# in3otd/glfer

Measured on AMD Instinct MI355X. Metric: spectrogram frames/sec + achieved HBM GB/s, N=4096 MTM K=4, higher is better.
Workload: dtype f32

## Files before the change

### glfer_amd/api.py

```python
import ctypes as C
import os

import numpy as np

_HERE = os.path.dirname(os.path.abspath(__file__))
LIB_PATH = os.environ.get("GLFER_LIB_PATH") or os.path.join(_HERE, "lib", "libglfer_hip.so")

MODE_FFT, MODE_MTM, MODE_HPARMA, MODE_LMP = 0, 1, 2, 3
WAV_PARTIAL_TAIL = 1
WINDOWS = {"hanning": 0, "blackman": 1, "gaussian": 2, "welch": 3,
           "bartlett": 4, "rectangular": 5, "hamming": 6, "kaiser": 7}
SAMPLES_F32, SAMPLES_S16, SAMPLES_U8 = 0, 1, 2
HISTORY_ZERO_FIRST, HISTORY_ZERO_ALWAYS = 0, 1
SUBMEAN_OFF, SUBMEAN_EXACT, SUBMEAN_FAST = 0, 1, 2
AVG_SUMAVG, AVG_PLAIN, AVG_SUMEXTREME = 1, 2, 3

EXPORTS = [
    "glfer_hip_plan_create", "glfer_hip_plan_destroy", "glfer_hip_hop", "glfer_hip_bins",
    "glfer_hip_num_tapers", "glfer_hip_num_frames", "glfer_hip_get_window", "glfer_hip_get_tapers",
    "glfer_hip_make_window", "glfer_hip_make_dpss", "glfer_hip_spectrogram_device",
    "glfer_hip_spectrum_device", "glfer_hip_spectrogram_host", "glfer_hip_wav_probe",
    "glfer_hip_spectrogram_wav", "glfer_hip_submean_device",
    "glfer_hip_floor_device",
    "glfer_hip_avg_device", "glfer_hip_palette", "glfer_hip_display_device", "glfer_hip_strerror", "glfer_hip_last_hip_error", "glfer_hip_version",
    "glfer_hip_frame_range", "glfer_hip_prepare_device", "glfer_hip_mtm_ftest_device", "glfer_hip_host_alloc",
    "glfer_hip_host_free", "glfer_hip_spectrogram_host_multi", "glfer_hip_spectrogram_wav_ex",
    "glfer_hip_avg_cum_device", "glfer_hip_waterfall_host", "glfer_hip_waterfall_device",
    "glfer_hip_spectrogram_host_workers",
    "glfer_hip_scratch_trim", "glfer_hip_scratch_held", "glfer_hip_scratch_limit", "glfer_hip_spectrogram_wav_range",
    "glfer_hip_spectrogram_wav_multi", "glfer_hip_spectrogram_wav_workers", "glfer_hip_levels_host",
    "glfer_hip_waterfall_map_device", "glfer_hip_waterfall_host_workers", "glfer_hip_waterfall_wav_workers",
    "glfer_hip_waterfall_wav_multi", "glfer_hip_submean_exact_device",
    "glfer_hip_numa_node_of_bus_id", "glfer_hip_numa_node_cpus", "glfer_hip_floor_device_pitched",
    "glfer_hip_abi_version", "glfer_hip_spectrogram_avg_device", "glfer_hip_workers_create", "glfer_hip_workers_destroy",
    "glfer_hip_workers_spectrogram_wav", "glfer_hip_workers_spectrogram_host",
    "glfer_hip_spectrogram_batch_device", "glfer_hip_avg_batch_device", "glfer_hip_spectrogram_avg_batch_device",
    "glfer_hip_waterfall_batch_device",
]


class GlferHipError(RuntimeError):
    pass


class Config(C.Structure):
    _fields_ = [("mode", C.c_int), ("n", C.c_int), ("overlap", C.c_float),
                ("window_type", C.c_int), ("limiter_a", C.c_float), ("enable_limiter", C.c_int),
                ("sub_mean", C.c_int), ("history_mode", C.c_int), ("mtm_w", C.c_float),
                ("mtm_k", C.c_int), ("sample_format", C.c_int), ("device", C.c_int),
                ("hparma_t", C.c_int), ("hparma_p_e", C.c_int), ("lmp_av", C.c_int), ("psd_pitch", C.c_int)]


class Display(C.Structure):
    _fields_ = [("scale_type", C.c_int), ("autoscale", C.c_int), ("overlap", C.c_float),
                ("max_level_db", C.c_float), ("min_level_db", C.c_float), ("thr_level", C.c_float),
                ("palette", C.c_int), ("first_buffer", C.c_int), ("display_max_lvl", C.c_float),
                ("display_min_lvl", C.c_float), ("psd_pitch", C.c_int)]

    def __init__(self, scale_type=2, autoscale=1, overlap=0.0, max_level_db=-10.0, min_level_db=-60.0,
                 thr_level=0.0, palette=0, first_buffer=1, psd_pitch=0):
        super().__init__(scale_type, autoscale, overlap, max_level_db, min_level_db, thr_level,
                         palette, first_buffer, 0.0, 0.0, psd_pitch)


SCALE_LIN, SCALE_LIN_MAX0, SCALE_LOG, SCALE_LOG_MAX0 = range(4)
PALETTES = {"hsv": 0, "thresh": 1, "cool": 2, "hot": 3, "bw": 4, "bone": 5, "copper": 6, "otd": 7}


class Phases(C.Structure):
    _fields_ = [("setup_s", C.c_double), ("read_s", C.c_double), ("h2d_s", C.c_double), ("kernel_s", C.c_double),
                ("d2h_s", C.c_double), ("wall_s", C.c_double), ("chunks", C.c_uint)]

    def as_dict(self):
        return {k: getattr(self, k) for k, _ in self._fields_}


class WavInfo(C.Structure):
    _fields_ = [("format", C.c_int), ("channels", C.c_int), ("sample_rate", C.c_int),
                ("bits_per_sample", C.c_int), ("data_offset", C.c_size_t), ("nsamples", C.c_size_t),
                ("data_bytes", C.c_size_t)]


_lib = None


def lib():
    global _lib
    if _lib is not None:
        return _lib
    try:
        import torch
    except ImportError:
        pass
    if not os.path.exists(LIB_PATH):
        raise GlferHipError(
            "HIP extension not built: %s is missing (run `python -c 'import __graft_entry__ as g; "
            "g.build()'` or `make -C glfer_amd/csrc`). There is no CPU fallback." % LIB_PATH)
    L = C.CDLL(LIB_PATH)
    vp, sz = C.c_void_p, C.c_size_t
    L.glfer_hip_plan_create.argtypes = [C.POINTER(Config), C.POINTER(vp)]
    L.glfer_hip_plan_destroy.argtypes = [vp]
    L.glfer_hip_plan_destroy.restype = None
    for f in ("glfer_hip_hop", "glfer_hip_bins", "glfer_hip_num_tapers"):
        getattr(L, f).argtypes = [vp]
    L.glfer_hip_num_frames.argtypes = [vp, sz]
    L.glfer_hip_num_frames.restype = sz
    L.glfer_hip_get_window.argtypes = [vp, vp]
    L.glfer_hip_get_tapers.argtypes = [vp, vp, vp]
    L.glfer_hip_make_window.argtypes = [C.c_int, C.c_int, vp]
    L.glfer_hip_make_dpss.argtypes = [C.c_int, C.c_int, C.c_double, vp, vp]
    L.glfer_hip_spectrogram_device.argtypes = [vp, vp, sz, sz, sz, vp, vp]
    L.glfer_hip_spectrogram_batch_device.argtypes = [vp, vp, sz, sz, sz, sz, sz, vp, vp]
    L.glfer_hip_spectrum_device.argtypes = [vp, vp, sz, sz, sz, vp, vp, vp]
    L.glfer_hip_spectrogram_host.argtypes = [vp, vp, sz, vp, C.POINTER(sz)]
    L.glfer_hip_wav_probe.argtypes = [C.c_char_p, C.POINTER(WavInfo)]
    L.glfer_hip_spectrogram_wav.argtypes = [vp, C.c_char_p, vp, sz, C.POINTER(sz), sz]
    L.glfer_hip_submean_device.argtypes = [vp, vp, C.c_int, sz, C.c_int, vp]
    L.glfer_hip_submean_exact_device.argtypes = [vp, vp, C.c_int, sz, C.c_int, vp]
    L.glfer_hip_floor_device.argtypes = [vp, sz, C.c_int, vp, vp]
    L.glfer_hip_floor_device_pitched.argtypes = [vp, sz, C.c_int, C.c_int, vp, vp]
    L.glfer_hip_palette.argtypes = [C.c_int, vp]
    L.glfer_hip_display_device.argtypes = [C.POINTER(Display), vp, vp, vp, sz, C.c_int, vp, vp, vp, vp]
    L.glfer_hip_avg_device.argtypes = [C.c_int, vp, sz, C.c_int, C.c_int, C.c_int, C.c_int, C.c_int,
                                       C.c_int, vp, vp, vp]
    L.glfer_hip_frame_range.argtypes = [sz, C.c_uint, C.c_uint, C.POINTER(sz), C.POINTER(sz)]
    L.glfer_hip_frame_range.restype = None
    L.glfer_hip_prepare_device.argtypes = [vp, vp, sz, sz, sz, vp, vp]
    L.glfer_hip_mtm_ftest_device.argtypes = [vp, vp, sz, sz, sz, vp, C.c_int, vp]
    L.glfer_hip_host_alloc.argtypes = [sz]
    L.glfer_hip_host_alloc.restype = vp
    L.glfer_hip_host_free.argtypes = [vp]
    L.glfer_hip_host_free.restype = None
    L.glfer_hip_spectrogram_host_multi.argtypes = [C.POINTER(Config), C.c_uint, vp, sz, vp, C.POINTER(sz)]
    L.glfer_hip_spectrogram_host_workers.argtypes = [C.POINTER(Config), C.POINTER(C.c_int), C.c_int, vp, sz, vp, C.POINTER(sz)]
    L.glfer_hip_spectrogram_wav_ex.argtypes = [vp, C.c_char_p, vp, sz, C.POINTER(sz), sz, C.c_uint]
    L.glfer_hip_avg_cum_device.argtypes = [vp, sz, C.c_int, C.c_int, C.c_int, C.c_int, C.c_int, vp, vp]
    L.glfer_hip_waterfall_device.argtypes = [C.POINTER(Display), C.c_int, C.c_int, C.c_int, C.c_int, C.c_int, vp, sz, C.c_int,
                                             vp, vp, vp, vp]
    L.glfer_hip_waterfall_host.argtypes = [vp, C.POINTER(Display), vp, sz, vp, vp, C.POINTER(sz)]
    cfgp, ip, dispp, szp = C.POINTER(Config), C.POINTER(C.c_int), C.POINTER(Display), C.POINTER(sz)
    L.glfer_hip_spectrogram_wav_range.argtypes = [vp, C.c_char_p, sz, sz, vp, szp, sz, C.c_uint]
    L.glfer_hip_spectrogram_wav_multi.argtypes = [cfgp, C.c_uint, C.c_char_p, vp, sz, szp, C.c_uint]
    L.glfer_hip_spectrogram_wav_workers.argtypes = [cfgp, ip, C.c_int, C.c_char_p, vp, sz, szp, C.c_uint]
    L.glfer_hip_waterfall_host_workers.argtypes = [cfgp, ip, C.c_int, dispp, C.c_int, C.c_int, C.c_int, C.c_int, C.c_int,
                                                   vp, sz, vp, vp, szp]
    L.glfer_hip_waterfall_wav_workers.argtypes = [cfgp, ip, C.c_int, dispp, C.c_int, C.c_int, C.c_int, C.c_int, C.c_int,
                                                  C.c_char_p, sz, vp, vp, szp, C.c_uint]
    L.glfer_hip_waterfall_wav_multi.argtypes = [cfgp, C.c_uint, dispp, C.c_int, C.c_int, C.c_int, C.c_int, C.c_int,
                                                C.c_char_p, sz, vp, vp, szp, C.c_uint]
    L.glfer_hip_levels_host.argtypes = [dispp, vp, sz, vp, C.c_int]
    L.glfer_hip_waterfall_map_device.argtypes = [dispp, C.c_int, C.c_int, C.c_int, C.c_int, C.c_int, vp, sz, sz, C.c_int,
                                                 vp, vp, vp, vp]
    L.glfer_hip_numa_node_of_bus_id.argtypes = [C.c_char_p, C.c_char_p]
    L.glfer_hip_numa_node_cpus.argtypes = [C.c_int, C.c_char_p, vp, sz]
    L.glfer_hip_scratch_trim.argtypes = [C.c_int, sz]
    L.glfer_hip_scratch_trim.restype = sz
    L.glfer_hip_scratch_held.argtypes = [C.c_int]
    L.glfer_hip_scratch_held.restype = sz
    L.glfer_hip_scratch_limit.argtypes = [sz]
    L.glfer_hip_scratch_limit.restype = None
    for f in ("glfer_hip_strerror", "glfer_hip_last_hip_error", "glfer_hip_version"):
        getattr(L, f).restype = C.c_char_p
    L.glfer_hip_strerror.argtypes = [C.c_int]
    L.glfer_hip_abi_version.argtypes = []
    L.glfer_hip_workers_create.argtypes = [C.POINTER(Config), C.POINTER(C.c_int), C.c_int, sz, C.POINTER(vp)]
    L.glfer_hip_workers_destroy.argtypes = [vp]
    L.glfer_hip_workers_destroy.restype = None
    L.glfer_hip_workers_spectrogram_wav.argtypes = [vp, C.c_char_p, vp, sz, C.POINTER(sz), C.c_uint, C.POINTER(Phases)]
    L.glfer_hip_workers_spectrogram_host.argtypes = [vp, vp, sz, vp, C.POINTER(sz), C.POINTER(Phases)]
    L.glfer_hip_spectrogram_avg_device.argtypes = [vp, vp, sz, sz, sz, C.c_int, C.c_int, C.c_int, C.c_int, C.c_int, C.c_int, vp, vp, vp, vp]
    L.glfer_hip_waterfall_batch_device.argtypes = [dispp, sz, C.c_int, C.c_int, C.c_int, C.c_int, C.c_int, vp, sz, C.c_int, vp, vp,
                                                   vp, vp]
    L.glfer_hip_avg_batch_device.argtypes = [C.c_int, vp, sz, sz, C.c_int, C.c_int, C.c_int, C.c_int, C.c_int, C.c_int, vp, vp, vp]
    L.glfer_hip_spectrogram_avg_batch_device.argtypes = [vp, vp, sz, sz, sz, sz, sz, C.c_int, C.c_int, C.c_int, C.c_int, C.c_int,
                                                         C.c_int, vp, vp, vp, vp]
    _lib = L
    return L


def _check(rc, what):
    if rc != 0:
        L = lib()
        raise GlferHipError("%s failed: %s (%s)" % (
            what, L.glfer_hip_strerror(rc).decode(), L.glfer_hip_last_hip_error().decode()))


def version():
    return lib().glfer_hip_version().decode()


def make_window(window_type, n):
    w = np.empty(n, np.float32)
    _check(lib().glfer_hip_make_window(int(window_type), n, w.ctypes.data), "make_window")
    return w


def make_dpss(n, kmax, nw):
    v = np.empty((kmax + 1, n), np.float64)
    s = np.empty(kmax + 1, np.float64)
    _check(lib().glfer_hip_make_dpss(n, kmax, float(nw), v.ctypes.data, s.ctypes.data), "make_dpss")
    return v, s


class FftParams:

    def __init__(self, n=1024, window_type=7, overlap=0.0, a=0.0, limiter=0, sub_mean=0,
                 history_mode=HISTORY_ZERO_FIRST, sample_format=SAMPLES_F32, psd_pitch=0):
        self.mode = MODE_FFT
        self.psd_pitch = psd_pitch
        self.n, self.window_type, self.overlap = n, window_type, overlap
        self.a, self.limiter, self.sub_mean = a, limiter, sub_mean
        self.history_mode, self.sample_format = history_mode, sample_format
        self.w, self.kmax = 0.0, 0


class MtmParams:

    def __init__(self, n=1024, overlap=0.0, w=4.0, kmax=7, sub_mean=0,
                 history_mode=HISTORY_ZERO_FIRST, sample_format=SAMPLES_F32, psd_pitch=0):
        self.mode = MODE_MTM
        self.psd_pitch = psd_pitch
        self.n, self.overlap, self.w, self.kmax = n, overlap, w, kmax
        self.window_type = WINDOWS["rectangular"]
        self.a, self.limiter, self.sub_mean = 0.0, 0, sub_mean
        self.history_mode, self.sample_format = history_mode, sample_format


class HparmaParams:

    def __init__(self, n=4096, overlap=0.0, t=96, p_e=16, sub_mean=0, history_mode=HISTORY_ZERO_FIRST,
                 sample_format=SAMPLES_F32):
        self.mode = MODE_HPARMA
        self.n, self.overlap, self.t, self.p_e = n, overlap, t, p_e
        self.window_type = WINDOWS["rectangular"]
        self.a, self.limiter, self.sub_mean = 0.0, 0, sub_mean
        self.history_mode, self.sample_format = history_mode, sample_format
        self.w, self.kmax = 0.0, 0


class LmpParams:

    def __init__(self, n=1024, overlap=0.0, avg=4, sub_mean=0, history_mode=HISTORY_ZERO_FIRST,
                 sample_format=SAMPLES_F32):
        self.mode = MODE_LMP
        self.n, self.overlap, self.avg = n, overlap, avg
        self.window_type = WINDOWS["rectangular"]
        self.a, self.limiter, self.sub_mean = 0.0, 0, sub_mean
        self.history_mode, self.sample_format = history_mode, sample_format
        self.w, self.kmax = 0.0, 0


_TORCH_DTYPES = None


def _torch():
    import torch
    return torch


def make_config(params, device=0):
    return Config(params.mode, params.n, params.overlap, params.window_type, params.a,
                  params.limiter, params.sub_mean, params.history_mode, params.w, params.kmax,
                  params.sample_format, device, getattr(params, "t", 0), getattr(params, "p_e", 0),
# ... 438 lines not shown
```

### glfer_amd/csrc/glfer_hip.cpp

```cpp
#include "plan.h"

#include <algorithm>
#include <cmath>
#include <cstdlib>
#include <cstdio>
#include <cstring>
#include <map>
#include <mutex>
#include <new>

#include "host_tables.h"
#include "spectro_params.h"

extern "C" hipError_t glfer_launch_hparma(const SpectroParams *sp, int n, int t, int ncol, const int *rot_sched, int rot_steps, int rot_width, const uint16_t *lagmap,
                                          const float2 *unit, hipStream_t st);
extern "C" hipError_t glfer_launch_floor(const float *psd, size_t nframes, int bins, int pitch, int m, float *stats,
                                         hipStream_t st);
extern "C" hipError_t glfer_launch_avg(int mode, const float *psd, size_t nframes, int bins, int n_out,
                                       int depth, int minbin, int maxbin, int max0, double *avg,
                                       double *ret, hipStream_t st);
extern "C" hipError_t glfer_launch_avg_batch(int mode, const float *psd, size_t nframes, int bins, int n_out, int depth, int minbin,
                                             int maxbin, int max0, double *avg, double *ret, unsigned nb, long long psd_bs,
                                             long long avg_bs, long long ret_bs, hipStream_t st);
extern "C" int glfer_avgmap_applies(size_t walk, int bins, int depth, int minbin, int maxbin);
// ... 149 lines not shown
      } else if (!b.out && b.cap >= want && (!best || b.cap < best->cap)) {
        best = &b;
      }
    }
    if (!best && !empty) {
      BigBlock *victim = nullptr;
      for (BigBlock &b : ds.big)
        if (!b.out && b.cap < want && (!victim || b.cap < victim->cap)) victim = &b;
      if (victim) {
        drop_block(*victim);
        empty = victim;
      }
    }
    if (!best && empty) {
      size_t held = 0;
      for (BigBlock &b : ds.big)
        if (b.p) held += b.cap;
      if (held + want > g_scratch_cap) trim_locked(ds, g_scratch_cap > want ? g_scratch_cap - want : 0);
      void *q = nullptr;
      hipEvent_t ev = nullptr;
      hipError_t me = hipMalloc(&q, want);
      if (me != hipSuccess) {
        (void)hipGetLastError();
        q = nullptr;
        if (trim_locked(ds, 0) > 0) me = hipMalloc(&q, want);
        for (BigBlock &b : ds.big)
          if (!b.p) { empty = &b; break; }
      }
      if (me == hipSuccess && hipEventCreateWithFlags(&ev, hipEventDisableTiming) == hipSuccess) {
        empty->p = q;
        empty->cap = want;
        empty->freed = ev;
        empty->used = false;
        empty->dev = dev;
        best = empty;
      } else {
        (void)hipGetLastError();
        if (q) (void)hipFree(q);
      }
    }
    if (best) {
      best->out = true;
      hipError_t e = hipSuccess;
      if (best->used && best->last != st) e = hipStreamWaitEvent(st, best->freed, 0);
      if (e != hipSuccess) {
        best->out = false;
        return e;
      }
      *p = best->p;
      return hipSuccess;
    }
  }
  lock.unlock();
  return hipMallocAsync(p, bytes, st);
}

void scratch_free(void *q, hipStream_t st) {
  if (!q) return;
  {
    std::lock_guard<std::mutex> lock(g_scratch_mu);
    for (DeviceScratch &ds : g_scratch)
      for (BigBlock &b : ds.big)
        if (b.p == q) {
          int cur = -1;
          const bool moved = hipGetDevice(&cur) == hipSuccess && cur != b.dev && b.dev >= 0 && hipSetDevice(b.dev) == hipSuccess;
          if (hipEventRecord(b.freed, st) == hipSuccess) {
            b.used = true;
            b.last = st;
          } else {
            (void)hipGetLastError();
            if (hipStreamSynchronize(st) != hipSuccess) {
              (void)hipGetLastError();
              (void)hipDeviceSynchronize();
              (void)hipFree(b.p);
              (void)hipEventDestroy(b.freed);
              b = BigBlock();
              if (moved) (void)hipSetDevice(cur);
              return;
            }
            b.used = false;
            b.last = nullptr;
          }
          b.out = false;
          if (b.dev >= 0 && b.dev < 64) trim_locked(g_scratch[b.dev], g_scratch_cap);
          if (moved) (void)hipSetDevice(cur);
          return;
        }
  }
  (void)hipFreeAsync(q, st);
}

size_t scratch_trim(int dev, size_t keep_bytes) {
  if (dev < 0 || dev >= 64) return 0;
  DeviceGuard guard(dev);
  std::lock_guard<std::mutex> lock(g_scratch_mu);
  return trim_locked(g_scratch[dev], keep_bytes);
}
size_t scratch_held(int dev) {
  if (dev < 0 || dev >= 64) return 0;
  std::lock_guard<std::mutex> lock(g_scratch_mu);
  size_t held = 0;
  for (BigBlock &b : g_scratch[dev].big)
    if (b.p) held += b.cap;
  return held;
}
void scratch_set_cap(size_t bytes) {
  std::lock_guard<std::mutex> lock(g_scratch_mu);
  g_scratch_cap = bytes;
  int cur = -1;
  if (hipGetDevice(&cur) != hipSuccess) cur = -1;
  for (int dev = 0; dev < 64; dev++) {
    size_t held = 0;
    for (BigBlock &b : g_scratch[dev].big)
      if (b.p) held += b.cap;
    if (held <= bytes) continue;
    if (dev != cur && hipSetDevice(dev) != hipSuccess) { (void)hipGetLastError(); continue; }
    trim_locked(g_scratch[dev], bytes);
    if (dev != cur && cur >= 0) (void)hipSetDevice(cur);
  }
}

hipError_t allow_dynamic_lds(const void *kernel, size_t bytes) {
  static std::mutex mu;
  static std::map<std::pair<int, const void *>, size_t> allowed;
  int dev = 0;
  hipError_t e = hipGetDevice(&dev);
  if (e != hipSuccess) return e;
  std::lock_guard<std::mutex> lock(mu);
  size_t &have = allowed[{dev, kernel}];
  if (bytes <= have) return hipSuccess;
  e = hipFuncSetAttribute(kernel, hipFuncAttributeMaxDynamicSharedMemorySize, (int)bytes);
  if (e == hipSuccess) have = bytes;
  return e;
}

}
using glfer::DeviceGuard;
using glfer::hip_fail;

static int data_device(const void *d_ptr) {
  int dev = glfer::device_of(d_ptr);
  if (dev < 0 && hipGetDevice(&dev) != hipSuccess) dev = 0;
  return dev;
}

static bool is_pow2(int n) { return n > 0 && (n & (n - 1)) == 0; }

static size_t tap_slot(int n, int pair, int i, int which) {
  if (n < 256) return ((size_t)pair * n + i) * 2 + which;
  const int T = n / 16, t = i % T, m = i / T;
  return (size_t)pair * n * 2 + ((size_t)(m / 2) * T + t) * 4 + (size_t)(m & 1) * 2 + which;
}

extern "C" {

const char *glfer_hip_version(void) { return "glfer_hip 0.9 (gfx950; 16 points/lane Stockham radix-16 with LDS exchange, inter-pass twiddles folded into the butterflies: packed pairs, real-input and wavefront-private forms, shared odd taper, register reuse across overlapped frames, mean removal in the reference's summation order (cfg.sub_mean = 1) or inside the kernels; N = 8..1048576; periodogram, multitaper + F-test, HP-ARMA with column-disjoint Jacobi rotations side by side and frames from a queue, LMP; rows at a caller's pitch; wavefront floor, fused average, display map with the average taken inside it; chunk ring for ingest with uploads and downloads at once, WAV files and waterfalls over several GPUs, read-ahead behind the per-hop shim, kept scratch blocks with a cap, workers bound to their GPU's NUMA node)"; }

int glfer_hip_abi_version(void) { return GLFER_HIP_ABI; }

int glfer_hip_palette(int palette, unsigned char colortab[768]) {
  if (!colortab) return GLFER_E_ARG;
  glfer::make_palette(palette, colortab);
  return GLFER_OK;
}

}

struct MapAverages {
  int mode, depth, minbin, maxbin, max0;
  const float *d_batch;
  size_t first;
};

static int display_columns(glfer_hip_display *d, const float *d_psd, const double *d_avg, const MapAverages *fused,
                           const float *d_stats, size_t nframes, int bins, unsigned char *d_rgb, short *d_lev,
                           float *d_levels, void *hip_stream, const float *d_levels_in = nullptr, int psd_pitch = 0) {
  if (!d || (!d_stats && !d_levels_in) || !d_rgb || bins < 1) return GLFER_E_ARG;
  if (psd_pitch == 0) psd_pitch = bins;
  if (psd_pitch < bins || (fused && psd_pitch != bins)) return GLFER_E_ARG;
  if ((d_psd != nullptr) + (d_avg != nullptr) + (fused != nullptr) != 1) return GLFER_E_ARG;
  if (d->scale_type < GLFER_SCALE_LIN || d->scale_type > GLFER_SCALE_LOG_MAX0) return GLFER_E_ARG;
  if (nframes == 0) return GLFER_OK;
  hipStream_t st = (hipStream_t)hip_stream;
  DeviceGuard guard(data_device(d_rgb));
  HIP_TRY(guard.error());
  const int scale_log = d->scale_type == GLFER_SCALE_LOG || d->scale_type == GLFER_SCALE_LOG_MAX0;

  const size_t lev_floats = (d_levels || d_levels_in) ? 0 : nframes * 4;
  const size_t st_floats = (d->autoscale && !d_levels_in) ? glfer_levels_scratch_floats(nframes) : 0;
  const size_t thr_bytes = (2 * glfer::kLogThrK + 1) * sizeof(double);
  unsigned char *scratch = nullptr;
  HIP_TRY(glfer::scratch_malloc((void **)&scratch, 768 + thr_bytes + (lev_floats + st_floats) * sizeof(float), st));
  unsigned char *d_tab = scratch;
  double *d_thr = reinterpret_cast<double *>(scratch + 768);
  float *fs = reinterpret_cast<float *>(scratch + 768 + thr_bytes);
  float *levels = d_levels_in ? const_cast<float *>(d_levels_in) : (d_levels ? d_levels : fs);
  float *chunk_state = st_floats ? fs + lev_floats : nullptr;
  int rc = GLFER_OK;
  auto fail = [&](hipError_t err) { rc = hip_fail(err, "glfer_hip_display_device"); };
  unsigned char tab[768];
  glfer::make_palette(d->palette, tab);
  hipError_t e = hipMemcpyAsync(d_tab, tab, 768, hipMemcpyHostToDevice, st);
  if (e == hipSuccess) e = hipMemcpyAsync(d_thr, glfer::log_thresholds(), thr_bytes, hipMemcpyHostToDevice, st);
  if (e != hipSuccess) fail(e);

  if (rc == GLFER_OK && !d_levels_in) {
    if (d->autoscale) {
      e = glfer_launch_levels(d_stats, nframes, scale_log, 1, d->first_buffer, d->overlap, d->display_max_lvl,
                              d->display_min_lvl, levels, chunk_state, st);
    } else {
      float mx = pow(10.0, d->max_level_db / 10.0);
      float mn = pow(10.0, d->min_level_db / 10.0);
      mn = (mx > mn ? mn : mx / 10.0);
      const float dmax = scale_log ? (float)(10.0 * log10(mx)) : mx;
      const float dmin = scale_log ? (float)(10.0 * log10(mn)) : mn;
      e = glfer_launch_levels_fixed(nframes, dmax, dmin, mx, mn, levels, st);
    }
    if (e != hipSuccess) fail(e);
  }
  if (rc == GLFER_OK) {
    const float thr_level = d->thr_level / 100.0;
    if (fused)
      e = glfer_launch_avgmap(fused->mode, fused->d_batch, fused->first, fused->first + nframes, bins, fused->depth,
                              fused->minbin, fused->maxbin, fused->max0, scale_log, 255.0 * thr_level,
                              1.0 - thr_level, levels, d_tab, d_thr, d_rgb, d_lev, st);
    else
      e = glfer_launch_map(d_psd, d_avg, nframes, bins, psd_pitch, scale_log, 255.0 * thr_level, 1.0 - thr_level, levels,
                           d_tab, d_thr, d_rgb, d_lev, st);
    if (e != hipSuccess) fail(e);
  }
  float last[4] = {0, 0, 0, 0};
  if (rc == GLFER_OK && !d_levels_in) {
    e = hipMemcpyAsync(last, levels + (nframes - 1) * 4, sizeof last, hipMemcpyDeviceToHost, st);
    if (e != hipSuccess) fail(e);
  }
  glfer::scratch_free(scratch, st);
  e = hipStreamSynchronize(st);
  if (e != hipSuccess && rc == GLFER_OK) fail(e);
  if (rc == GLFER_OK && !d_levels_in) {
    d->display_max_lvl = last[2];
    d->display_min_lvl = last[3];
    if (d->autoscale) d->first_buffer = 0;
  }
  return rc;
}

extern "C" {

int glfer_hip_display_device(glfer_hip_display *d, const float *d_psd, const double *d_avg, const float *d_stats,
                             size_t nframes, int bins, unsigned char *d_rgb, short *d_lev, float *d_levels,
                             void *hip_stream) {
  if (!d || (d_psd == nullptr) == (d_avg == nullptr)) return GLFER_E_ARG;
  return display_columns(d, d_psd, d_avg, nullptr, d_stats, nframes, bins, d_rgb, d_lev, d_levels, hip_stream, nullptr, d->psd_pitch);
}

}

static void waterfall_route(int avg_mode, int depth, int minbin, int maxbin, int bins, int pitch, size_t nframes, bool *fused_out,
                            size_t *tile_out) {
  const bool averaging = avg_mode != 0;
  bool fused = averaging && pitch == bins;
  if (const char *e = getenv("GLFER_WATERFALL_FUSED")) fused = fused && atoi(e) != 0;
  size_t tile = (averaging && !fused) ? std::max<size_t>(16384, ((size_t)4 << 30) / ((size_t)bins * sizeof(double))) : (size_t)1 << 22;
  if (const char *e = getenv("GLFER_WATERFALL_TILE")) {
    const long v = atol(e);
    if (v >= 64) tile = (size_t)v;
  }
  tile = std::min(tile, nframes);
  tile = (nframes + (nframes + tile - 1) / tile - 1) / ((nframes + tile - 1) / tile);
  const size_t last_tile = nframes - (nframes - 1) / tile * tile;
  if (fused) fused = glfer_avgmap_applies(tile, bins, depth, minbin, maxbin) != 0 &&
                     glfer_avgmap_applies(last_tile, bins, depth, minbin, maxbin) != 0;
  *fused_out = fused;
  *tile_out = tile;
}

static int waterfall_columns(glfer_hip_display *d, int avg_mode, int depth, int minbin, int maxbin, int max0,
                             const float *d_batch, size_t row0, size_t nframes, int bins, unsigned char *d_rgb, short *d_lev,
                             float *d_stats, void *hip_stream, const float *d_levels_in, int pitch = 0) {
  if (pitch == 0) pitch = bins;
  const float *d_psd = d_batch ? d_batch + row0 * (size_t)pitch : nullptr;
  if (!d || !d_psd || !d_rgb || bins < 1 || bins > 32769 || pitch < bins) return GLFER_E_ARG;
  const bool averaging = avg_mode != 0;
  if (averaging && (avg_mode < GLFER_AVG_SUMAVG || avg_mode > GLFER_AVG_SUMEXTREME || depth < 1 || minbin < 0 ||
                    maxbin <= minbin || maxbin > bins))
    return GLFER_E_ARG;
  if (nframes == 0) return GLFER_OK;
  hipStream_t st = (hipStream_t)hip_stream;
  DeviceGuard guard(data_device(d_psd));
  HIP_TRY(guard.error());
  bool fused = false;
  size_t tile = 0;
  waterfall_route(avg_mode, depth, minbin, maxbin, bins, pitch, nframes, &fused, &tile);
  const size_t back = averaging ? (size_t)depth : 0;
  float *stats = d_stats;
  double *avg = nullptr, *ret = nullptr;
  if (!stats && !d_levels_in) HIP_TRY(glfer::scratch_malloc((void **)&stats, tile * 4 * sizeof(float), st));
  int rc = GLFER_OK;
  if (averaging && !fused) {
    hipError_t e = glfer::scratch_malloc((void **)&avg, (tile + back) * (size_t)bins * sizeof(double), st);
    if (e == hipSuccess) e = glfer::scratch_malloc((void **)&ret, (tile + back) * 4 * sizeof(double), st);
    if (e != hipSuccess) rc = hip_fail(e, "hipMallocAsync(waterfall tile)");
  }
  for (size_t f0 = 0; rc == GLFER_OK && f0 < nframes; f0 += tile) {
    const size_t nf = std::min(tile, nframes - f0);
    float *tstats = d_stats ? d_stats + f0 * 4 : stats;
// ... 237 lines not shown
  if (ret) glfer::scratch_free(ret, st);
  if (levels) glfer::scratch_free(levels, st);
  if (!d_stats && stats) glfer::scratch_free(stats, st);
  glfer::scratch_free(small, st);
  e = hipStreamSynchronize(st);
  if (e != hipSuccess) fail(e, "glfer_hip_waterfall_batch_device");
  if (rc == GLFER_OK) {
    for (size_t b = 0; b < nstreams; b++) {
      if (autoscale) {
        disps[b].display_max_lvl = back_state[b * 3 + 1];
        disps[b].display_min_lvl = back_state[b * 3 + 2];
        disps[b].first_buffer = 0;
      } else {
        disps[b].display_max_lvl = mx;
        disps[b].display_min_lvl = mn;
      }
    }
  }
  return rc;
}

size_t glfer_hip_scratch_trim(int device, size_t keep_bytes) {
  size_t ring = 0;
  if (keep_bytes == 0 && device >= 0 && device < 64) {
    DeviceGuard guard(device);
    if (guard.error() == hipSuccess) {
      ring = glfer::workers_kept_bytes(device);
      glfer::workers_drop_kept();
      ring += glfer::ingest_ring_spare_bytes(device);
      glfer::ingest_ring_drop_spare(device);
    }
  }
  return ring + glfer::scratch_trim(device, keep_bytes);
}
size_t glfer_hip_scratch_held(int device) { return glfer::scratch_held(device) + glfer::ingest_ring_spare_bytes(device) + glfer::workers_kept_bytes(device); }
void glfer_hip_scratch_limit(size_t bytes) {
  glfer::scratch_set_cap(bytes);
  if (bytes == 0) glfer::workers_drop_kept();
  int cur = -1;
  if (hipGetDevice(&cur) != hipSuccess) cur = -1;
  for (int dev = 0; dev < 64; dev++)
    if (glfer::ingest_ring_spare_bytes(dev) > bytes) {
      DeviceGuard guard(dev);
      if (guard.error() == hipSuccess) glfer::ingest_ring_drop_spare(dev);
    }
}

const char *glfer_hip_strerror(int code) {
  switch (code) {
    case GLFER_OK: return "ok";
    case GLFER_E_ARG: return "bad argument or unsupported configuration";
    case GLFER_E_HIP: return "HIP runtime error";
    case GLFER_E_NOMEM: return "out of memory";
    case GLFER_E_NUMERIC: return "DPSS eigen-solve did not converge";
  }
  return "unknown error";
}

const char *glfer_hip_last_hip_error(void) { return g_hip_err.c_str(); }

int glfer_hip_plan_create(const glfer_hip_config *cfg, glfer_hip_plan **out) {
  if (!cfg || !out) return GLFER_E_ARG;
  *out = nullptr;
  const int n = cfg->n;
  if (!is_pow2(n) || n < 8 || n > (1 << 20)) return GLFER_E_ARG;
  if (cfg->mode == GLFER_MODE_HPARMA && (n < 32 || n > 32768)) return GLFER_E_ARG;
  const bool small = n < 256, huge = n > 16384;
  if (!(cfg->overlap >= 0.0f) || !(cfg->overlap < 1.0f)) return GLFER_E_ARG;
  if (cfg->mode != GLFER_MODE_FFT && cfg->mode != GLFER_MODE_MTM && cfg->mode != GLFER_MODE_HPARMA &&
      cfg->mode != GLFER_MODE_LMP)
    return GLFER_E_ARG;
  if (cfg->mode == GLFER_MODE_LMP && (cfg->lmp_av < 1 || cfg->lmp_av > 4096)) return GLFER_E_ARG;
  if (cfg->mode == GLFER_MODE_HPARMA) {
    const int t = cfg->hparma_t, ncol = cfg->hparma_p_e + 1;
    if (t < 2 || ncol < 2 || ncol > t || t > n || ncol > 256 || t > 65535) return GLFER_E_ARG;
    const size_t xlen = (size_t)n + (t <= 128 ? 128 : 0);
    const size_t big = xlen > (size_t)t * ncol ? xlen : (size_t)t * ncol;
    if ((big + (size_t)ncol * ncol + t + 2 * ncol) * sizeof(float) > 160 * 1024) return GLFER_E_ARG;
  }
  if (cfg->sample_format < 0 || cfg->sample_format > 2) return GLFER_E_ARG;
  if (cfg->mode == GLFER_MODE_MTM && (cfg->mtm_k < 0 || cfg->mtm_k > 31 || !(cfg->mtm_w > 0.0f)))
    return GLFER_E_ARG;
  if (cfg->mode == GLFER_MODE_FFT && (cfg->window_type < 0 || cfg->window_type > 7)) return GLFER_E_ARG;

  glfer_hip_plan *p = new (std::nothrow) glfer_hip_plan();
  if (!p) return GLFER_E_NOMEM;
  p->cfg = *cfg;
  p->n = n;
  p->hop = (int)(n * (1.0 - cfg->overlap));
  p->keep = n - p->hop;
  p->bins = n / 2 + 1;
  p->lanes = n / 64;
  if (p->hop <= 0) { delete p; return GLFER_E_ARG; }
  p->pitch = cfg->psd_pitch ? cfg->psd_pitch : p->bins;
  if (cfg->psd_pitch < 0 || p->pitch < p->bins || (cfg->psd_pitch && cfg->mode == GLFER_MODE_LMP)) { delete p; return GLFER_E_ARG; }

  p->window.assign(n, 1.0f);
  std::vector<float> taps;
  const bool lmp = cfg->mode == GLFER_MODE_LMP;
  if (lmp) {
    p->cfg.window_type = GLFER_WIN_RECTANGULAR;
    p->cfg.limiter_a = 0.0f;
    p->cfg.enable_limiter = 0;
    p->lmp_av = cfg->lmp_av;
  }
  if (cfg->mode == GLFER_MODE_FFT || lmp) {
    p->ntapers = 1;
    p->npairs = 1;
    glfer::make_window(p->cfg.window_type, n, p->window.data());
    p->nonlin = (p->cfg.limiter_a > 0.0f) || (p->cfg.enable_limiter == 1);
    const double scale = std::sqrt(1.0 / ((huge ? 4.0 : 2.0) * n));
    p->spec_unscale = (float)scale;
    taps.assign((size_t)2 * n, 0.0f);
    const bool rect = (p->cfg.window_type == GLFER_WIN_RECTANGULAR);
    for (int i = 0; i < n; i++) {
      const double w = rect ? 1.0 : (double)p->window[i];
      taps[tap_slot(n, 0, i, 0)] = p->nonlin ? (float)w : (float)(w * scale);
    }
  } else if (cfg->mode == GLFER_MODE_HPARMA) {
    p->ntapers = 0;
    p->npairs = 0;
    taps.assign(4, 0.0f);
  } else {
    p->ntapers = cfg->mtm_k + 1;
    p->npairs = (p->ntapers + 1) / 2;
    p->tapers.resize((size_t)p->ntapers * n);
    p->sig.resize(p->ntapers);
    {
      struct Kept { int n, kmax; float w; std::vector<double> tapers, sig; };
      static std::mutex mu;
      static std::vector<Kept> kept;
      bool hit = false;
      {
        std::lock_guard<std::mutex> lock(mu);
        for (const Kept &k : kept)
          if (k.n == n && k.kmax == cfg->mtm_k && k.w == cfg->mtm_w) {
            p->tapers = k.tapers;
            p->sig = k.sig;
            hit = true;
            break;
          }
      }
      if (!hit) {
        if (!glfer::make_dpss(n, cfg->mtm_k, (double)cfg->mtm_w, p->tapers.data(), p->sig.data())) {
          delete p;
          return GLFER_E_NUMERIC;
        }
        std::lock_guard<std::mutex> lock(mu);
        if (kept.size() >= 4) kept.erase(kept.begin());
        kept.push_back(Kept{n, cfg->mtm_k, cfg->mtm_w, p->tapers, p->sig});
      }
    }
    taps.assign((size_t)2 * p->npairs * n, 0.0f);
    for (int j = 0; j < p->ntapers && !huge; j++) {
      const double scale = std::sqrt(1.0 / (2.0 * n * (1.0 + p->sig[j])));
      for (int i = 0; i < n; i++)
        taps[tap_slot(n, j / 2, i, j & 1)] = (float)(p->tapers[(size_t)j * n + i] * scale);
    }
    p->spec_unscale = 1.0f;
  }
  int logn = 0;
  while ((1 << logn) < n) logn++;
  p->lanes = n / 16;
  std::vector<float> tw(2, 0.0f);
  if (!small && !huge) {
    tw.assign((size_t)2 * glfer::make_twiddles16(logn, nullptr) * p->lanes, 0.0f);
    glfer::make_twiddles16(logn, tw.data());
  }
  if (huge) taps.assign(4, 0.0f);

  std::vector<float> htaps, htw, hrot;
  const bool h_periodogram = (cfg->mode == GLFER_MODE_FFT || lmp) && !p->nonlin && n >= 512 && !huge;
  const bool h_multitaper = cfg->mode == GLFER_MODE_MTM && n >= 8192 && !huge;
  if (h_periodogram || h_multitaper) {
    const int th = n / 32;
    const int nwin = h_multitaper ? p->ntapers : 1;
    const bool rect = h_periodogram && (p->cfg.window_type == GLFER_WIN_RECTANGULAR);
    htaps.resize((size_t)nwin * n);
    for (int j = 0; j < nwin; j++) {
      const double scale = std::sqrt(1.0 / (4.0 * n * (h_multitaper ? 1.0 + p->sig[j] : 1.0)));
      for (int m = 0; m < 16; m++)
        for (int t = 0; t < th; t++)
          for (int e = 0; e < 2; e++) {
            const int i = 2 * (t + th * m) + e;
            const double w = h_multitaper ? p->tapers[(size_t)j * n + i] : (rect ? 1.0 : (double)p->window[i]);
            htaps[(size_t)j * n + ((size_t)(m / 2) * th + t) * 4 + (size_t)(m & 1) * 2 + e] = (float)(w * scale);
          }
    }
    p->htapers = nwin;
    htw.resize((size_t)2 * glfer::make_twiddles16(logn - 1, nullptr) * th);
    glfer::make_twiddles16(logn - 1, htw.data());
    hrot.resize((size_t)2 * th);
    for (int t = 0; t < th; t++) {
      const double ang = 2.0 * 3.14159265358979323846 * t / n;
      hrot[2 * t] = (float)std::cos(ang);
      hrot[2 * t + 1] = (float)std::sin(ang);
    }
  }

  std::vector<float> wtaps, wtw, wcomb;
  const bool w_form = (((cfg->mode == GLFER_MODE_FFT || lmp) && (!p->nonlin || huge)) || cfg->mode == GLFER_MODE_MTM) && n >= 2048;
  if (w_form) {
    const int M = n / 2, W = M / 1024, LF = 64 * W, IPL = LF <= 512 ? 512 / LF : 1;
    const bool mt = cfg->mode == GLFER_MODE_MTM;
    const int nwin = mt ? p->ntapers : 1;
    const bool rect = !mt && (p->cfg.window_type == GLFER_WIN_RECTANGULAR);
    wtaps.resize((size_t)nwin * n);
    for (int j = 0; j < nwin; j++) {
      const double scale = std::sqrt(1.0 / (4.0 * n * (mt ? 1.0 + p->sig[j] : 1.0)));
      for (int w = 0; w < W; w++)
        for (int m = 0; m < 16; m++)
          for (int t = 0; t < 64; t++)
            for (int e = 0; e < 2; e++) {
              const int i = 2 * (W * (t + 64 * m) + w) + e;
              const double v = mt ? p->tapers[(size_t)j * n + i] : (rect ? 1.0 : (double)p->window[i]);
              wtaps[((((size_t)j * W + w) * 8 + m / 2) * 64 + t) * 4 + (size_t)(m & 1) * 2 + e] = (float)(p->nonlin ? v : v * scale);
            }
    }
    p->wtapers = nwin;
    wtw.resize((size_t)2 * glfer::make_twiddles16(10, nullptr) * 64);
    glfer::make_twiddles16(10, wtw.data());
    wcomb.resize(n <= 32768 ? (size_t)2 * IPL * W * LF : 2);
    const double two_pi = 2.0 * 3.14159265358979323846;
    for (int i = 0; i < IPL && n <= 32768; i++)
      for (int ww = 0; ww < W; ww++)
        for (int u = 0; u < LF; u++) {
          const long long k1 = u + (long long)LF * i;
          const double ang = ww == 0 ? two_pi * (double)k1 / n : two_pi * (double)((ww * k1) % M) / M;
          wcomb[2 * ((size_t)(i * W + ww) * LF + u)] = (float)std::cos(ang);
          wcomb[2 * ((size_t)(i * W + ww) * LF + u) + 1] = (float)std::sin(ang);
        }
  }

  std::vector<float> xtaps;
  if (cfg->mode == GLFER_MODE_MTM && (p->ntapers & 1) && p->ntapers >= 3 && !small && !huge) {
    const int T = n / 16, j = p->ntapers - 1;
    const double scale = std::sqrt(1.0 / (4.0 * n * (1.0 + p->sig[j])));
    xtaps.resize((size_t)n);
    for (int i = 0; i < n; i++) {
      const int t = i % T, m = i / T;
      xtaps[((size_t)(m / 4) * T + t) * 4 + (size_t)(m & 3)] = (float)(p->tapers[(size_t)j * n + i] * scale);
    }
  }

  std::vector<float> ltaps;
  if (!xtaps.empty() && n <= 4096) {
    const int T = n / 16, nfull = p->npairs - 1;
    bool sym = true;
    for (int j = 0; j < p->ntapers && sym; j++) {
      const double *v = &p->tapers[(size_t)j * n];
      double peak = 0.0, dev = 0.0;
      for (int i = 0; i < n / 2; i++) {
        peak = std::max(peak, std::fabs(v[i]));
        dev = std::max(dev, std::fabs(v[n - 1 - i] - ((j & 1) ? -v[i] : v[i])));
      }
      sym = dev <= 1e-7 * peak;
    }
    const size_t lds = ((size_t)(n + n / 16) * (T >= 256 ? 1 : 256 / T) + 16 * 17 + 8 + (size_t)nfull * 8 * T + 4 * T) * 8;
    if (sym && lds <= 80 * 1024) {
      ltaps.resize((size_t)nfull * 8 * T * 2 + (size_t)8 * T);
      for (int j = 0; j < p->ntapers; j++) {
        const bool last = j == p->ntapers - 1;
        const double scale = std::sqrt(1.0 / ((last ? 4.0 : 2.0) * n * (1.0 + p->sig[j])));
        for (int m = 0; m < 8; m++)
          for (int t = 0; t < T; t++) {
            const float val = (float)(p->tapers[(size_t)j * n + t + T * m] * scale);
            if (last) ltaps[(size_t)nfull * 8 * T * 2 + (size_t)m * T + t] = val;
            else ltaps[(((size_t)(j / 2) * 8 + m) * T + t) * 2 + (j & 1)] = val;
          }
      }
    }
  }

  std::vector<uint16_t> lagmap;
  std::vector<float> unit;
  std::vector<int> rot_sched;
  if (cfg->mode == GLFER_MODE_HPARMA) {
    const int t = cfg->hparma_t, ncol = cfg->hparma_p_e + 1;
    const int width = [] { const char *e = getenv("GLFER_HPARMA_WIDTH"); return e && atoi(e) == 16 ? 16 : 8; }();
    p->rot_width = width;
    if (ncol >= 2 && ncol <= 64) {
      std::vector<std::pair<int, int>> rots;
      for (int j = 0; j < ncol - 1; j++)
        for (int k = j + 1; k < ncol; k++) rots.push_back({j, k});
      const int R = (int)rots.size();
      std::vector<std::vector<int>> succ(R);
      std::vector<int> indeg(R, 0), lastc(ncol, -1), lp(R, 1);
      for (int i = 0; i < R; i++) {
        const int cs[2] = {rots[i].first, rots[i].second};
        int seen = -1;
        for (int c : cs) {
          if (lastc[c] >= 0 && lastc[c] != seen) {
            succ[lastc[c]].push_back(i);
            indeg[i]++;
            seen = lastc[c];
          }
          lastc[c] = i;
        }
      }
      for (int i = R - 1; i >= 0; i--)
        for (int s : succ[i]) lp[i] = std::max(lp[i], 1 + lp[s]);
      std::vector<int> ready;
      for (int i = 0; i < R; i++)
        if (!indeg[i]) ready.push_back(i);
      int done = 0;
      while (done < R) {
        std::sort(ready.begin(), ready.end(), [&](int a, int b) { return lp[a] != lp[b] ? lp[a] > lp[b] : a < b; });
        const int take = std::min<int>(width, (int)ready.size());
        std::vector<int> cur(ready.begin(), ready.begin() + take);
        ready.erase(ready.begin(), ready.begin() + take);
        for (int g = 0; g < width; g++) rot_sched.push_back(g < take ? (rots[cur[g]].first | rots[cur[g]].second << 8) : -1);
        for (int i : cur) {
          done++;
          for (int s : succ[i])
            if (--indeg[s] == 0) ready.push_back(s);
        }
      }
    }
    std::vector<int> flat((size_t)(t + 1) * ncol, -1);
    for (int i = 0; i < t; i++) flat[i] = i;
    for (int i = 1; i < t; i++)
      for (int j = 0; j < ncol; j++) flat[(size_t)i * ncol + j] = flat[std::abs(j - i)];
    lagmap.resize((size_t)t * ncol);
    for (size_t i = 0; i < lagmap.size(); i++) lagmap[i] = (uint16_t)(flat[i] < 0 ? 0 : flat[i]);
    unit.resize((size_t)2 * (n / 2 + 1));
    for (int k = 0; k <= n / 2; k++) {
      const double ang = -2.0 * 3.14159265358979323846 * k / n;
      unit[2 * k] = (float)std::cos(ang);
      unit[2 * k + 1] = (float)std::sin(ang);
    }
  }

  DeviceGuard guard(cfg->device);
  hipError_t e = guard.error();
  if (e == hipSuccess) e = hipMalloc((void **)&p->d_taps, taps.size() * sizeof(float));
  if (e == hipSuccess && cfg->mode == GLFER_MODE_FFT && cfg->window_type != GLFER_WIN_RECTANGULAR) {
    e = hipMalloc((void **)&p->d_window, (size_t)n * sizeof(float));
    if (e == hipSuccess) e = hipMemcpy(p->d_window, p->window.data(), (size_t)n * sizeof(float), hipMemcpyHostToDevice);
  }
  if (e == hipSuccess) e = hipMalloc((void **)&p->d_tw, tw.size() * sizeof(float));
  if (e == hipSuccess) e = hipMemcpy(p->d_taps, taps.data(), taps.size() * sizeof(float), hipMemcpyHostToDevice);
  if (e == hipSuccess) e = hipMemcpy(p->d_tw, tw.data(), tw.size() * sizeof(float), hipMemcpyHostToDevice);
  if (e == hipSuccess && !htaps.empty()) {
    e = hipMalloc((void **)&p->d_htaps, htaps.size() * sizeof(float));
    if (e == hipSuccess) e = hipMalloc((void **)&p->d_htw, htw.size() * sizeof(float));
    if (e == hipSuccess) e = hipMalloc((void **)&p->d_hrot, hrot.size() * sizeof(float));
    if (e == hipSuccess) e = hipMemcpy(p->d_htaps, htaps.data(), htaps.size() * sizeof(float), hipMemcpyHostToDevice);
    if (e == hipSuccess) e = hipMemcpy(p->d_htw, htw.data(), htw.size() * sizeof(float), hipMemcpyHostToDevice);
    if (e == hipSuccess) e = hipMemcpy(p->d_hrot, hrot.data(), hrot.size() * sizeof(float), hipMemcpyHostToDevice);
  }
  if (e == hipSuccess && !wtaps.empty()) {
    e = hipMalloc((void **)&p->d_wtaps, wtaps.size() * sizeof(float));
    if (e == hipSuccess) e = hipMalloc((void **)&p->d_wtw, wtw.size() * sizeof(float));
    if (e == hipSuccess) e = hipMalloc((void **)&p->d_wcomb, wcomb.size() * sizeof(float));
    if (e == hipSuccess) e = hipMemcpy(p->d_wtaps, wtaps.data(), wtaps.size() * sizeof(float), hipMemcpyHostToDevice);
    if (e == hipSuccess) e = hipMemcpy(p->d_wtw, wtw.data(), wtw.size() * sizeof(float), hipMemcpyHostToDevice);
    if (e == hipSuccess) e = hipMemcpy(p->d_wcomb, wcomb.data(), wcomb.size() * sizeof(float), hipMemcpyHostToDevice);
    if (e == hipSuccess && huge) {
      const int M = n / 2, W = M / 1024;
      std::vector<float> bt((size_t)W * 16 * 2);
      for (int w = 0; w < W; w++)
        for (int m = 0; m < 16; m++) {
          const double ang = -2.0 * 3.14159265358979323846 * (double)(((long long)64 * w * m) % M) / M;
          bt[2 * ((size_t)w * 16 + m)] = (float)std::cos(ang);
          bt[2 * ((size_t)w * 16 + m) + 1] = (float)std::sin(ang);
        }
      e = hipMalloc((void **)&p->d_bigtw, bt.size() * sizeof(float));
      if (e == hipSuccess) e = hipMemcpy(p->d_bigtw, bt.data(), bt.size() * sizeof(float), hipMemcpyHostToDevice);
    }
  }
  if (e == hipSuccess && !xtaps.empty()) {
    e = hipMalloc((void **)&p->d_xtaps, xtaps.size() * sizeof(float));
    if (e == hipSuccess) e = hipMemcpy(p->d_xtaps, xtaps.data(), xtaps.size() * sizeof(float), hipMemcpyHostToDevice);
  }
  if (e == hipSuccess && !ltaps.empty()) {
    e = hipMalloc((void **)&p->d_ltaps, ltaps.size() * sizeof(float));
    if (e == hipSuccess) e = hipMemcpy(p->d_ltaps, ltaps.data(), ltaps.size() * sizeof(float), hipMemcpyHostToDevice);
  }
  if (e == hipSuccess && !lagmap.empty()) {
    e = hipMalloc((void **)&p->d_lagmap, lagmap.size() * sizeof(uint16_t));
    if (e == hipSuccess) e = hipMalloc((void **)&p->d_unit, unit.size() * sizeof(float));
    if (e == hipSuccess) e = hipMemcpy(p->d_lagmap, lagmap.data(), lagmap.size() * sizeof(uint16_t), hipMemcpyHostToDevice);
    if (e == hipSuccess && !rot_sched.empty()) {
      e = hipMalloc((void **)&p->d_rot_sched, rot_sched.size() * sizeof(int));
      if (e == hipSuccess) e = hipMemcpy(p->d_rot_sched, rot_sched.data(), rot_sched.size() * sizeof(int), hipMemcpyHostToDevice);
      p->rot_steps = (int)(rot_sched.size() / p->rot_width);
    }
    if (e == hipSuccess) e = hipMemcpy(p->d_unit, unit.data(), unit.size() * sizeof(float), hipMemcpyHostToDevice);
  }
  if (e != hipSuccess) {
    int rc = hip_fail(e, "plan_create");
    glfer_hip_plan_destroy(p);
    return rc;
  }
  *out = p;
  return GLFER_OK;
}

void glfer_hip_plan_destroy(glfer_hip_plan *p) {
  if (!p) return;
  DeviceGuard guard(p->cfg.device);
  if (p->d_taps) (void)hipFree(p->d_taps);
  if (p->d_window) (void)hipFree(p->d_window);
  if (p->d_ftaps_mu_first) (void)hipFree(p->d_ftaps_mu_first);
  if (p->d_ftaps2) (void)hipFree(p->d_ftaps2);
  if (p->d_U0) (void)hipFree(p->d_U0);
  if (p->d_tw) (void)hipFree(p->d_tw);
  if (p->d_htaps) (void)hipFree(p->d_htaps);
  if (p->d_htw) (void)hipFree(p->d_htw);
  if (p->d_hrot) (void)hipFree(p->d_hrot);
  if (p->d_xtaps) (void)hipFree(p->d_xtaps);
  if (p->d_wtaps) (void)hipFree(p->d_wtaps);
  if (p->d_wtw) (void)hipFree(p->d_wtw);
  if (p->d_wcomb) (void)hipFree(p->d_wcomb);
  if (p->d_bigtw) (void)hipFree(p->d_bigtw);
  if (p->d_ltaps) (void)hipFree(p->d_ltaps);
  if (p->d_lagmap) (void)hipFree(p->d_lagmap);
  if (p->d_rot_sched) (void)hipFree(p->d_rot_sched);
  if (p->d_unit) (void)hipFree(p->d_unit);
  glfer::ingest_ring_free(p->ring);
  for (hipStream_t a : p->aux)
    if (a) (void)hipStreamDestroy(a);
  for (hipEvent_t ev : p->aux_events) (void)hipEventDestroy(ev);
  delete p;
}

int glfer_hip_hop(const glfer_hip_plan *p) { return p ? p->hop : GLFER_E_ARG; }
int glfer_hip_bins(const glfer_hip_plan *p) { return p ? p->bins : GLFER_E_ARG; }
int glfer_hip_num_tapers(const glfer_hip_plan *p) { return p ? p->ntapers : GLFER_E_ARG; }
size_t glfer_hip_num_frames(const glfer_hip_plan *p, size_t nsamples) {
  return p ? nsamples / (size_t)p->hop : 0;
}

int glfer_hip_get_window(const glfer_hip_plan *p, float *w) {
  if (!p || !w) return GLFER_E_ARG;
  memcpy(w, p->window.data(), (size_t)p->n * sizeof(float));
  return GLFER_OK;
}

int glfer_hip_get_tapers(const glfer_hip_plan *p, double *tapers, double *sig) {
  if (!p || p->cfg.mode != GLFER_MODE_MTM) return GLFER_E_ARG;
  if (tapers) memcpy(tapers, p->tapers.data(), p->tapers.size() * sizeof(double));
  if (sig) memcpy(sig, p->sig.data(), p->sig.size() * sizeof(double));
  return GLFER_OK;
}

int glfer_hip_make_window(int window_type, int n, float *window) {
  if (!window || n < 2 || window_type < 0 || window_type > 7) return GLFER_E_ARG;
  glfer::make_window(window_type, n, window);
  return GLFER_OK;
}

int glfer_hip_make_dpss(int n, int kmax, double nw, double *tapers, double *sig) {
  if (!tapers || !sig || n < 2 || kmax < 0 || kmax > 31 || !(nw > 0.0)) return GLFER_E_ARG;
  return glfer::make_dpss(n, kmax, nw, tapers, sig) ? GLFER_OK : GLFER_E_NUMERIC;
}

extern "C" hipError_t glfer_launch_spectro_small(const SpectroParams *p, int n, const float *staps, hipStream_t st);
extern "C" hipError_t glfer_launch_spectro16w_n15(const SpectroParams *p, hipStream_t st);
extern "C" hipError_t glfer_launch_spectro_big(const SpectroParams *p, int n, hipStream_t st);

static hipError_t launch_packed(const SpectroParams &sp, int n, hipStream_t st) {
  if (n < 256) return glfer_launch_spectro_small(&sp, n, sp.taps, st);
  switch (n) {
    case 256: return glfer_launch_spectro16_n8(&sp, st);
    case 512: return glfer_launch_spectro16_n9(&sp, st);
    case 1024: return glfer_launch_spectro16_n10(&sp, st);
    case 2048: return glfer_launch_spectro16_n11(&sp, st);
    case 4096: return glfer_launch_spectro16_n12(&sp, st);
    case 8192: return glfer_launch_spectro16_n13(&sp, st);
    case 16384: return glfer_launch_spectro16_n14(&sp, st);
  }
  return hipErrorInvalidValue;
}

static hipError_t launch_real_input(const SpectroParams &sp, int n, hipStream_t st) {
  switch (n) {
    case 512: return glfer_launch_spectro16h_n9(&sp, st);
    case 1024: return glfer_launch_spectro16h_n10(&sp, st);
    case 2048: return glfer_launch_spectro16h_n11(&sp, st);
    case 4096: return glfer_launch_spectro16h_n12(&sp, st);
    case 8192: return glfer_launch_spectro16h_n13(&sp, st);
    case 16384: return glfer_launch_spectro16h_n14(&sp, st);
  }
  return hipErrorInvalidValue;
}

#define GLFER_W_PERIODOGRAM(n) (false)
#define GLFER_W_MULTITAPER(n, tapers) ((n) >= 16384)

static int form_override();

static hipError_t launch_wave_private(const SpectroParams &sp, int n, hipStream_t st) {
  switch (n) {
    case 2048: return glfer_launch_spectro16w_n11(&sp, st);
    case 4096: return glfer_launch_spectro16w_n12(&sp, st);
    case 8192: return glfer_launch_spectro16w_n13(&sp, st);
    case 16384: return glfer_launch_spectro16w_n14(&sp, st);
    case 32768: return (sp.spec || form_override() == 'w') ? glfer_launch_spectro16w_n15(&sp, st) : glfer_launch_spectro_big(&sp, n, st);
    case 65536: return glfer_launch_spectro_big(&sp, n, st);
  }
  if (n >= 131072 && n <= (1 << 20)) return glfer_launch_spectro_big(&sp, n, st);
  return hipErrorInvalidValue;
}

static int form_override() {
  const char *e = getenv("GLFER_FORM");
  return e && *e ? (int)*e : 0;
}

static hipError_t launch_shared_odd(const SpectroParams &sp, int n, hipStream_t st) {
  if (n == 4096) return glfer_launch_spectro16y_n12(&sp, st);
  if (sp.ltaps) {
    switch (n) {
      case 256: return glfer_launch_spectro16xl_n8(&sp, st);
      case 512: return glfer_launch_spectro16xl_n9(&sp, st);
      case 1024: return glfer_launch_spectro16xl_n10(&sp, st);
      case 2048: return glfer_launch_spectro16xl_n11(&sp, st);
    }
  }
  switch (n) {
    case 256: return glfer_launch_spectro16x_n8(&sp, st);
    case 512: return glfer_launch_spectro16x_n9(&sp, st);
    case 1024: return glfer_launch_spectro16x_n10(&sp, st);
  }
  return hipErrorInvalidValue;
}

enum BodyRoute { ROUTE_PACKED, ROUTE_REAL_INPUT, ROUTE_SHARED_ODD, ROUTE_WAVE_PRIVATE };
static BodyRoute body_route(const SpectroParams &sp, int n) {
  const unsigned esz = sp.fmt == GLFER_FMT_F32 ? 4u : (sp.fmt == GLFER_FMT_S16 ? 2u : 1u);
  const bool pairs_aligned = sp.fmt == GLFER_FMT_F32 ||
                             ((sp.H & 1) == 0 && (reinterpret_cast<uintptr_t>(sp.stream) & (2u * esz - 1u)) == 0);
  const int force = form_override();
  bool real_input = sp.htaps && (sp.npairs == 1 || sp.htapers > 1) && n >= 512 && pairs_aligned;
  bool shared_odd = sp.xtaps && sp.npairs >= 2 && (sp.ltaps || n <= 1024 || n == 4096);
  bool wave_private = sp.wtaps && n >= 2048 && pairs_aligned &&
                      (force == 'w' || (force == 0 && (sp.npairs == 1 ? GLFER_W_PERIODOGRAM(n) : GLFER_W_MULTITAPER(n, sp.wtapers))));
  if (force == 'h') wave_private = false;
  if (force == 'x') wave_private = real_input = false;
  if (wave_private) real_input = true, shared_odd = false;
  if (sp.spec || sp.nonlin || !(real_input || shared_odd)) return ROUTE_PACKED;
  if (wave_private) return ROUTE_WAVE_PRIVATE;
  return real_input ? ROUTE_REAL_INPUT : ROUTE_SHARED_ODD;
}
static bool route_takes_mean(BodyRoute r, const SpectroParams &sp, int n) {
  if (n < 256 || n > 16384 || sp.spec || sp.nonlin || sp.history_mode) return false;
  if ((16 * sp.H) % n) return false;
  const int k16 = 16 * sp.H / n;
  switch (r) {
    case ROUTE_PACKED: return k16 == 4 || k16 == 8 || k16 == 16;
    case ROUTE_REAL_INPUT: return (sp.npairs == 1 && sp.htapers <= 1 && (k16 == 2 || k16 == 4 || k16 == 8 || k16 == 16)) ||
                                  (sp.htapers > 1 && n >= 8192 && k16 == 16);
    case ROUTE_SHARED_ODD: return (n == 4096 || n <= 1024) && (k16 == 4 || k16 == 8 || k16 == 16);
    case ROUTE_WAVE_PRIVATE: return sp.wtapers > 1 && (k16 == 8 || k16 == 16);
    default: return false;
  }
}

static bool route_takes_table(BodyRoute r, const SpectroParams &sp, int n) {
  switch (r) {
    case ROUTE_PACKED: return true;
    case ROUTE_REAL_INPUT: return true;
    case ROUTE_SHARED_ODD: return true;
    case ROUTE_WAVE_PRIVATE: return true;
    default: return false;
  }
}

static hipError_t launch_by_n(const SpectroParams &sp, int n, hipStream_t st) {
  if (n > 16384) return launch_wave_private(sp, n, st);
  const BodyRoute route = body_route(sp, n);
  const bool real_input = route == ROUTE_REAL_INPUT || route == ROUTE_WAVE_PRIVATE, wave_private = route == ROUTE_WAVE_PRIVATE;
  if (sp.mean_inkernel && !route_takes_mean(route, sp, n)) return hipErrorInvalidValue;
  if (route == ROUTE_PACKED) return launch_packed(sp, n, st);
  const long long first_inside = ((long long)sp.R + sp.H - 1) / sp.H;
  if (sp.mean_inkernel && sp.frame0 < first_inside) return hipErrorInvalidValue;
  const int lanes = n / 16;
  const long long G = real_input ? 1 : 2 * (lanes >= 256 ? 1 : 256 / lanes);
  const long long lo = sp.frame0, hi = sp.frame0 + sp.nframes;
  long long b0 = lo > first_inside ? lo : first_inside;
  b0 = (b0 + G - 1) / G * G;
  long long b1 = hi / G * G;
  if (sp.mean_inkernel && (b0 != lo || b1 != hi)) return hipErrorInvalidValue;
  if (b0 >= b1) return launch_packed(sp, n, st);
  auto sub = [&](long long from, long long to) {
    SpectroParams q = sp;
    q.frame0 = from;
    q.nframes = (int)(to - from);
    q.psd = sp.psd + (size_t)(from - lo) * (size_t)sp.pitch;
    q.mean_inkernel = 0;
    q.means = nullptr;
    return q;
  };
  if (b0 > lo) {
    const SpectroParams head = sub(lo, b0);
    hipError_t e = launch_packed(head, n, st);
    if (e != hipSuccess) return e;
  }
  if (hi > b1) {
    const SpectroParams tail = sub(b1, hi);
    hipError_t e = launch_packed(tail, n, st);
    if (e != hipSuccess) return e;
  }
  SpectroParams body = sub(b0, b1);
  body.mean_inkernel = sp.mean_inkernel;
  body.means = sp.means;
  if (wave_private) return launch_wave_private(body, n, st);
  return real_input ? launch_real_input(body, n, st) : launch_shared_odd(body, n, st);
}

}

static void fill_params(const glfer_hip_plan *p, SpectroParams &sp) {
  memset(&sp, 0, sizeof sp);
  sp.H = p->hop;
  sp.R = p->keep;
  sp.npairs = p->npairs;
  sp.history_mode = p->cfg.history_mode ? 1 : 0;
  sp.pitch = p->pitch;
  sp.fmt = p->cfg.sample_format;
  sp.nonlin = p->nonlin ? 1 : 0;
  sp.limiter = (p->cfg.enable_limiter == 1);
  sp.a = p->cfg.limiter_a;
  sp.post_scale = p->spec_unscale;
  sp.spec_unscale = p->spec_unscale;
  sp.taps = p->d_taps;
  sp.tw = p->d_tw;
  sp.htaps = p->d_htaps;
  sp.htapers = p->htapers;
  sp.htw = p->d_htw;
  sp.hrot = p->d_hrot;
  sp.xtaps = p->d_xtaps;
  sp.ltaps = p->d_ltaps;
  sp.wtaps = p->d_wtaps;
  sp.wtapers = p->wtapers;
  sp.wtw = p->d_wtw;
  sp.wcomb = p->d_wcomb;
  sp.bigtw = p->d_bigtw;
}

static bool reference_means(const glfer_hip_plan *p) { return p->cfg.sub_mean != 0 && p->cfg.sub_mean != GLFER_SUBMEAN_FAST; }

static int submean_scratch(const glfer_hip_plan *p, SpectroParams &sp, size_t first, size_t nframes, hipStream_t st,
                           float **scratch_out, long tail_fresh = -1) {
  const size_t hops_back = sp.history_mode ? 0 : (size_t)((p->keep + p->hop - 1) / p->hop);
  size_t hop_lo = (first > hops_back) ? first - hops_back : 0;
  const size_t last = first + nframes - 1;
  if (tail_fresh >= 0 && last > 0 && hop_lo > last - 1) hop_lo = last - 1;
  const size_t nhops = first + nframes - hop_lo;
  float *scratch = nullptr;
  HIP_TRY(glfer::scratch_malloc((void **)&scratch, nhops * (size_t)p->hop * sizeof(float), st));
  const size_t esz = sp.fmt == GLFER_FMT_F32 ? 4 : (sp.fmt == GLFER_FMT_S16 ? 2 : 1);
  const char *src = (const char *)sp.stream + hop_lo * (size_t)p->hop * esz;
  const bool exact = reference_means(p);
  float *means = nullptr;
  hipError_t e = hipSuccess;
  if (exact) {
    e = glfer::scratch_malloc((void **)&means, nhops * sizeof(float), st);
    if (e == hipSuccess) e = glfer_launch_hop_means_seq(src, means, p->hop, (long long)nhops, sp.fmt, st);
  }
  if (e == hipSuccess) e = glfer_launch_submean(src, scratch, p->hop, (long long)nhops, sp.fmt, st, means);
  if (e == hipSuccess && tail_fresh >= 0)
    e = glfer_launch_submean_tail_ex(src + (nhops - 1) * (size_t)p->hop * esz, nhops > 1 ? scratch + (nhops - 2) * (size_t)p->hop : nullptr,
                                     scratch + (nhops - 1) * (size_t)p->hop, p->hop, (int)tail_fresh, exact ? 1 : 0, sp.fmt, st);
  if (means) glfer::scratch_free(means, st);
  if (e != hipSuccess) {
    glfer::scratch_free(scratch, st);
    return hip_fail(e, "glfer_launch_submean");
  }
  sp.stream = reinterpret_cast<const char *>(scratch) - hop_lo * (size_t)p->hop * sizeof(float);
  sp.fmt = GLFER_FMT_F32;
  *scratch_out = scratch;
  return GLFER_OK;
}

static bool mean_inkernel_ok(const glfer_hip_plan *p, const SpectroParams &sp, const float *d_spec, long tail_fresh) {
  if (p->nonlin || d_spec || tail_fresh >= 0 || sp.history_mode) return false;
  if (p->cfg.mode != GLFER_MODE_FFT && p->cfg.mode != GLFER_MODE_LMP && p->cfg.mode != GLFER_MODE_MTM) return false;
  const char *e = getenv("GLFER_MEAN_PREPASS");
  if (e && *e == '1') return false;
  const BodyRoute r = body_route(sp, p->n);
  if (!route_takes_mean(r, sp, p->n)) return false;
  if (reference_means(p) && !route_takes_table(r, sp, p->n)) return false;
  return true;
}

static hipError_t launch_reference_means(const glfer_hip_plan *p, const SpectroParams &sp, size_t hop_lo, size_t nhops, float *means,
                                         unsigned blocks, hipStream_t st) {
  const size_t esz = sp.fmt == GLFER_FMT_F32 ? 4 : (sp.fmt == GLFER_FMT_S16 ? 2 : 1);
  const char *src = (const char *)sp.stream + hop_lo * (size_t)p->hop * esz;
  const int forced = [] { const char *e = getenv("GLFER_MEANS_HPW"); return e && *e ? atoi(e) : 0; }();
  int hpw = forced;
  if (!hpw) hpw = nhops >= 262144 ? (p->hop <= 2048 ? 16 : 64) : (nhops >= 32768 || p->hop % 1024 != 0 ? 16 : 4);
  if (hpw == 4 && p->hop % 1024 != 0) hpw = 16;
  if (hpw == 16 && p->hop % 256 != 0) hpw = 64;
  if ((hpw == 16 || hpw == 4) && (reinterpret_cast<uintptr_t>(src) & (4 * esz - 1)) == 0)
    return glfer_launch_hop_means_tiled(src, means, p->hop, (long long)nhops, sp.fmt, hpw, blocks, st);
  return glfer_launch_hop_means_seq(src, means, p->hop, (long long)nhops, sp.fmt, st);
}

static int launch_body_with_reference_means(glfer_hip_plan *p, const SpectroParams &bs, size_t b0, size_t b1, hipStream_t st) {
  const long piece_mb = [] { const char *e = getenv("GLFER_EXACT_PIECE_MB"); return e && *e ? atol(e) : 0L; }();
  const int nstreams_env = [] {
    const char *e = getenv("GLFER_EXACT_STREAMS");
    const int v = e && *e ? atoi(e) : 2;
    return v < 1 ? 1 : (v > 3 ? 3 : v);
  }();
  const unsigned means_blocks = [] { const char *e = getenv("GLFER_MEANS_BLOCKS"); return e && *e ? (unsigned)atol(e) : 0u; }();
  const size_t hops_back = (size_t)((p->keep + p->hop - 1) / p->hop);
  const size_t hop_lo = b0 - hops_back, nhops = b1 - hop_lo;
  const size_t esz = bs.fmt == GLFER_FMT_F32 ? 4 : (bs.fmt == GLFER_FMT_S16 ? 2 : 1);
  size_t piece = b1 - b0;
  if (piece_mb > 0) {
    piece = ((size_t)piece_mb << 20) / ((size_t)p->hop * esz);
    piece = std::max<size_t>(piece / 64 * 64, 64);
  }
  const size_t npieces = (b1 - b0 + piece - 1) / piece;
  int nstreams = npieces > 1 ? nstreams_env : 1;
  float *means = nullptr;
  hipError_t e = glfer::scratch_malloc((void **)&means, nhops * sizeof(float), st);
  if (e != hipSuccess) return hip_fail(e, "scratch (hop means)");
  SpectroParams q = bs;
  q.means = means - hop_lo;
  {
    const long producers = [] { const char *e = getenv("GLFER_MEANS_PRODUCERS"); return e && *e ? atol(e) : 0L; }();
    const bool periodogram_table = body_route(bs, p->n) == ROUTE_REAL_INPUT && bs.npairs == 1 && bs.htapers <= 1 && p->n <= 8192;
    const long min_frames = [] { const char *e = getenv("GLFER_FUSED_MIN_FRAMES"); return e && *e ? atol(e) : 65536L; }();
    if (producers > 0 && periodogram_table && npieces == 1 && (long)(b1 - b0) >= min_frames) {
      const long block_frames = [] { const char *e = getenv("GLFER_FUSED_BLOCK_FRAMES"); return e && *e ? atol(e) : 0L; }();
      const long look = [] { const char *e = getenv("GLFER_FUSED_LOOK"); return e && *e ? atol(e) : 1024L; }();
      const bool lockstep = block_frames > 0;
      const int chunk = lockstep ? 64 : 4096;
      const size_t nchunks = (nhops + chunk - 1) / chunk;
      unsigned *ready = nullptr;
      e = glfer::scratch_malloc((void **)&ready, (nchunks + 8) * sizeof(unsigned), st);
      if (e == hipSuccess) e = hipMemsetAsync(ready, 0, (nchunks + 8) * sizeof(unsigned), st);
      if (e == hipSuccess) {
        q.nprod = (int)(producers / 8 * 8);
        q.prod_chunk = chunk;
        q.means_out = means - hop_lo;
        q.means_ready = ready;
        q.prod_hop0 = (long long)hop_lo;
        q.prod_nhops = (long long)nhops;
        if (lockstep) {
          q.prod_front_frames = -1;
          q.prod_block_frames = (int)block_frames;
          q.prod_look = (int)look;
          q.front_done = ready + nchunks;
        }
        e = launch_by_n(q, p->n, st);
      }
      if (ready) glfer::scratch_free(ready, st);
      glfer::scratch_free(means, st);
      return e == hipSuccess ? GLFER_OK : hip_fail(e, "estimator launch (hop means produced in the launch)");
    }
  }
  static std::mutex aux_mu;
  bool own_aux = false;
  if (nstreams > 1) {
    std::lock_guard<std::mutex> lock(aux_mu);
    if (p->aux_busy) {
      nstreams = 1;
    } else {
      for (int i = 0; i < nstreams - 1 && e == hipSuccess; i++)
        if (!p->aux[i]) e = hipStreamCreateWithFlags(&p->aux[i], hipStreamNonBlocking);
      while (e == hipSuccess && p->aux_events.size() < 2 * npieces + 1) {
        hipEvent_t ev = nullptr;
        e = hipEventCreateWithFlags(&ev, hipEventDisableTiming);
        if (e == hipSuccess) p->aux_events.push_back(ev);
      }
      if (e != hipSuccess) {
        (void)hipGetLastError();
        nstreams = 1;
        e = hipSuccess;
      } else {
        p->aux_busy = own_aux = true;
      }
    }
  }
  if (nstreams <= 1) {
    for (size_t c = 0; c < npieces && e == hipSuccess; c++) {
      const size_t f0 = b0 + c * piece, f1 = std::min(b1, f0 + piece);
      const size_t h0 = c == 0 ? hop_lo : f0;
      e = launch_reference_means(p, bs, h0, f1 - h0, means + (h0 - hop_lo), 0, st);
      q.frame0 = (long long)f0;
      q.nframes = (int)(f1 - f0);
// ... 255 lines not shown
  const size_t esz = fmt == GLFER_FMT_F32 ? 4 : (fmt == GLFER_FMT_S16 ? 2 : 1);
  if (fmt != GLFER_FMT_F32 && (stream_pitch & 1)) return GLFER_E_ARG;
  const size_t rows = (size_t)p->pitch;
  if (stream_pitch > (SIZE_MAX / esz) / nstreams || nframes > (SIZE_MAX / sizeof(float) / rows) / nstreams) return GLFER_E_ARG;
  return batch_rows(p, d_streams, nstreams, stream_pitch, nsamples, first, nframes, d_psd, nframes * rows, (hipStream_t)hip_stream);
}

static int batch_rows(glfer_hip_plan *p, const void *d_streams, size_t nstreams, size_t stream_pitch, size_t nsamples, size_t first,
                      size_t nframes, float *d_psd, size_t psd_bs, hipStream_t st) {
  const int fmt = p->cfg.sample_format;
  const size_t esz = fmt == GLFER_FMT_F32 ? 4 : (fmt == GLFER_FMT_S16 ? 2 : 1);
  const char *base = static_cast<const char *>(d_streams);
  if (!batch_one_launch(p) || nstreams == 1) {
    for (size_t b = 0; b < nstreams; b++) {
      const int rc = glfer_run_device(p, base + b * stream_pitch * esz, nsamples, first, nframes, d_psd + b * psd_bs, nullptr, st);
      if (rc != GLFER_OK) return rc;
    }
    return GLFER_OK;
  }
  DeviceGuard guard(p->cfg.device);
  HIP_TRY(guard.error());
  int dev = 0, ymax = 0;
  HIP_TRY(hipGetDevice(&dev));
  HIP_TRY(hipDeviceGetAttribute(&ymax, hipDeviceAttributeMaxGridDimY, dev));
  ymax = std::max(1, std::min(ymax, 65535));
  for (size_t c0 = 0; c0 < nstreams; c0 += (size_t)ymax) {
    const unsigned nb = (unsigned)std::min(nstreams - c0, (size_t)ymax);
    SpectroParams sp;
    fill_params(p, sp);
    sp.stream = base + c0 * stream_pitch * esz;
    sp.frame0 = (long long)first;
    sp.nframes = (int)nframes;
    sp.psd = d_psd + c0 * psd_bs;
    sp.nbatch = (int)nb;
    sp.batch_stride = (long long)(stream_pitch * esz);
    sp.psd_batch_stride = (long long)psd_bs;
    int rc = GLFER_OK;
    if (p->cfg.sub_mean && mean_inkernel_ok(p, sp, nullptr, -1)) {
      rc = batch_mean_inkernel(p, sp, first, nframes, nb, st);
    } else {
      float *scratch = nullptr;
      if (p->cfg.sub_mean) rc = batch_submean_scratch(p, sp, first, nframes, nb, st, &scratch);
      if (rc == GLFER_OK) {
        const hipError_t e = launch_by_n(sp, p->n, st);
        if (e != hipSuccess) rc = hip_fail(e, "estimator launch (batch)");
      }
      if (scratch) glfer::scratch_free(scratch, st);
    }
    if (rc != GLFER_OK) return rc;
  }
  return GLFER_OK;
}

int glfer_hip_spectrum_device(glfer_hip_plan *p, const void *d_stream, size_t nsamples, size_t first,
                              size_t nframes, float *d_psd, float *d_spec, void *hip_stream) {
  if (!d_spec) return GLFER_E_ARG;
  return glfer_run_device(p, d_stream, nsamples, first, nframes, d_psd, d_spec, (hipStream_t)hip_stream);
}

int glfer_hip_prepare_device(glfer_hip_plan *p, const void *d_stream, size_t nsamples, size_t first,
                             size_t nframes, float *d_frames, void *hip_stream) {
  if (!p || !d_stream || (!d_frames && nframes)) return GLFER_E_ARG;
  if (nframes == 0) return GLFER_OK;
  if ((first + nframes) > nsamples / (size_t)p->hop || nframes > 0x7fffffffu) return GLFER_E_ARG;
  hipStream_t st = (hipStream_t)hip_stream;
  DeviceGuard guard(p->cfg.device);
  HIP_TRY(guard.error());
  SpectroParams sp;
  fill_params(p, sp);
  sp.stream = d_stream;
  sp.frame0 = (long long)first;
  sp.nframes = (int)nframes;
  float *scratch = nullptr;
  int rc = GLFER_OK;
  if (p->cfg.sub_mean) rc = submean_scratch(p, sp, first, nframes, st, &scratch);
  if (rc == GLFER_OK) {
    hipError_t e = glfer_launch_prepare(&sp, p->n, p->d_window, d_frames, st);
    if (e != hipSuccess) rc = hip_fail(e, "glfer_launch_prepare");
  }
  if (scratch) glfer::scratch_free(scratch, st);
  return rc;
}

int glfer_hip_mtm_ftest_device(glfer_hip_plan *p, const void *d_stream, size_t nsamples, size_t first,
                               size_t nframes, float *d_ftest, int mu_live, void *hip_stream) {
  if (!p || !d_stream || (!d_ftest && nframes) || p->cfg.mode != GLFER_MODE_MTM) return GLFER_E_ARG;
  if (p->n > 16384) return GLFER_E_ARG;
  if (nframes == 0) return GLFER_OK;
  if ((first + nframes) > nsamples / (size_t)p->hop || nframes > 0x7fffffffu) return GLFER_E_ARG;
  hipStream_t st = (hipStream_t)hip_stream;
  DeviceGuard guard(p->cfg.device);
  HIP_TRY(guard.error());
  const int n = p->n, T = p->ntapers;
  if (!p->d_ftaps) {
    p->U0.resize(T);
    p->hn.resize(n);
    glfer::make_ftest_tables(n, T - 1, p->tapers.data(), p->U0.data(), p->hn.data(), &p->sum_U0_sqr);
    std::vector<float> taps((size_t)(T + 2) * 2 * n, 0.0f);
    for (int j = -1; j <= T; j++)
      for (int i = 0; i < n; i++)
        taps[(size_t)(j + 1) * 2 * n + tap_slot(n, 0, i, 0)] = (j >= 0 && j < T) ? (float)p->tapers[(size_t)j * n + i] : p->hn[i];
    float *d = nullptr;
    double *du = nullptr;
    HIP_TRY(hipMalloc((void **)&d, taps.size() * sizeof(float)));
    hipError_t e = hipMalloc((void **)&du, (size_t)T * sizeof(double));
    if (e == hipSuccess) e = hipMemcpy(d, taps.data(), taps.size() * sizeof(float), hipMemcpyHostToDevice);
    if (e == hipSuccess) e = hipMemcpy(du, p->U0.data(), (size_t)T * sizeof(double), hipMemcpyHostToDevice);
    if (e != hipSuccess) {
      (void)hipFree(d);
      (void)hipFree(du);
      return hip_fail(e, "ftest tables");
    }
    p->d_ftaps_mu_first = d;
    p->d_ftaps = d + (size_t)2 * n;
    p->d_U0 = du;
    {
      int ex = 0;
      (void)frexpf(sqrtf(p->sum_U0_sqr), &ex);
      p->hn_scale = p->sum_U0_sqr > 0.0f && ex > 0 && ex < 64 ? ldexpf(1.0f, ex - 1) : 1.0f;
    }
    const int r_mu = (T + 2) / 2, r_nomu = (T + 1) / 2;
    std::vector<float> pt((size_t)(r_mu + r_nomu) * 2 * n, 0.0f);
    auto seq = [&](int s_, int i, bool with_mu) -> float {
      const int j = with_mu ? s_ - 1 : s_;
      if (j >= T) return 0.0f;
      return 0.5f * (j < 0 ? p->hn_scale * p->hn[i] : (float)p->tapers[(size_t)j * n + i]);
    };
    for (int r = 0; r < r_mu + r_nomu; r++) {
      const bool with_mu = r < r_mu;
      const int rr = with_mu ? r : r - r_mu;
      for (int i = 0; i < n; i++) {
        pt[(size_t)r * 2 * n + tap_slot(n, 0, i, 0)] = seq(2 * rr, i, with_mu);
        pt[(size_t)r * 2 * n + tap_slot(n, 0, i, 1)] = seq(2 * rr + 1, i, with_mu);
      }
    }
    float *d2 = nullptr;
    hipError_t e2 = hipMalloc((void **)&d2, pt.size() * sizeof(float));
    if (e2 == hipSuccess) e2 = hipMemcpy(d2, pt.data(), pt.size() * sizeof(float), hipMemcpyHostToDevice);
    if (e2 != hipSuccess) {
      (void)hipFree(d2);
      return hip_fail(e2, "ftest tables (paired)");
    }
    p->d_ftaps2 = d2;
    p->d_ftaps2_nomu = d2 + (size_t)r_mu * 2 * n;
  }
  SpectroParams sp;
  fill_params(p, sp);
  sp.pitch = p->bins;
  sp.stream = d_stream;
  sp.npairs = 1;
  sp.nonlin = 0;
  sp.post_scale = sp.spec_unscale = 1.0f;
  sp.htaps = nullptr;
  sp.xtaps = sp.ltaps = nullptr;
  float *scratch = nullptr;
  int rc = GLFER_OK;
  if (p->cfg.sub_mean) {
    sp.frame0 = (long long)first;
    rc = submean_scratch(p, sp, first, nframes, st, &scratch);
  }
  if (rc == GLFER_OK && n >= 256) {
    SpectroParams q = sp;
    q.frame0 = (long long)first;
    q.nframes = (int)nframes;
    q.psd = nullptr;
    q.spec = nullptr;
    q.ftest = d_ftest;
    q.ft_U0 = p->d_U0;
    q.ft_sum_U0_sqr = p->sum_U0_sqr;
    q.ft_mu_live = mu_live ? 1 : 0;
    q.npairs = mu_live ? T + 1 : T;
    q.taps = mu_live ? p->d_ftaps_mu_first : p->d_ftaps;
    const char *pe = getenv("GLFER_FTEST_PAIRED");
    if (pe && *pe ? *pe != '0' : n >= 2048) {
      q.ft_nseq = mu_live ? T + 1 : T;
      q.npairs = (q.ft_nseq + 1) / 2;
      q.taps = mu_live ? p->d_ftaps2 : p->d_ftaps2_nomu;
      q.ft_mu_unscale = 1.0f / p->hn_scale;
    }
    hipError_t e = launch_packed(q, n, st);
    if (e != hipSuccess) rc = hip_fail(e, "ftest launch");
    if (scratch) glfer::scratch_free(scratch, st);
    return rc;
  }
  size_t group = ((size_t)256 << 20) / ((size_t)(T + 1) * n * sizeof(float));
  group = std::max<size_t>(1, std::min<size_t>(group, 32768));
  float *spec = nullptr, *dummy = nullptr;
  if (rc == GLFER_OK) {
    const size_t g = std::min(group, nframes);
    hipError_t e = glfer::scratch_malloc((void **)&spec, (size_t)(T + 1) * g * n * sizeof(float), st);
    if (e == hipSuccess) e = glfer::scratch_malloc((void **)&dummy, g * (size_t)p->bins * sizeof(float), st);
    if (e != hipSuccess) rc = hip_fail(e, "hipMallocAsync(ftest spectra)");
  }
  for (size_t done = 0; rc == GLFER_OK && done < nframes; done += group) {
    const size_t g = std::min(group, nframes - done);
    hipError_t e = hipSuccess;
    for (int j = 0; j <= T && e == hipSuccess; j++) {
      if (j == T && !mu_live) break;
      SpectroParams q = sp;
      q.frame0 = (long long)(first + done);
      q.nframes = (int)g;
      q.taps = p->d_ftaps + (size_t)j * 2 * n;
      q.psd = dummy;
      q.spec = spec + (size_t)j * g * n;
      e = launch_packed(q, n, st);
    }
    if (e == hipSuccess)
      e = glfer_launch_ftest(spec, g, n, T, p->d_U0, p->sum_U0_sqr, mu_live ? 1 : 0, d_ftest + done * (size_t)p->bins, st);
    if (e != hipSuccess) rc = hip_fail(e, "ftest launch");
  }
  if (spec) glfer::scratch_free(spec, st);
  if (dummy) glfer::scratch_free(dummy, st);
  if (scratch) glfer::scratch_free(scratch, st);
  return rc;
}

int glfer_hip_submean_device(const void *d_in, float *d_out, int hop, size_t nhops, int sample_format,
                             void *hip_stream) {
  if (!d_in || !d_out || hop < 1 || sample_format < 0 || sample_format > 2) return GLFER_E_ARG;
  DeviceGuard guard(data_device(d_out));
  HIP_TRY(guard.error());
  HIP_TRY(glfer_launch_submean(d_in, d_out, hop, (long long)nhops, sample_format, (hipStream_t)hip_stream, nullptr));
  return GLFER_OK;
}

int glfer_hip_submean_exact_device(const void *d_in, float *d_out, int hop, size_t nhops, int sample_format,
                                   void *hip_stream) {
  if (!d_in || !d_out || hop < 1 || sample_format < 0 || sample_format > 2) return GLFER_E_ARG;
  if (nhops == 0) return GLFER_OK;
  hipStream_t st = (hipStream_t)hip_stream;
  DeviceGuard guard(data_device(d_out));
  HIP_TRY(guard.error());
  float *means = nullptr;
  HIP_TRY(glfer::scratch_malloc((void **)&means, nhops * sizeof(float), st));
  hipError_t e = glfer_launch_hop_means_seq(d_in, means, hop, (long long)nhops, sample_format, st);
  if (e == hipSuccess) e = glfer_launch_submean(d_in, d_out, hop, (long long)nhops, sample_format, st, means);
  glfer::scratch_free(means, st);
  return e == hipSuccess ? GLFER_OK : hip_fail(e, "glfer_hip_submean_exact_device");
}

int glfer_hip_floor_device_pitched(const float *d_psd, size_t nframes, int bins, int pitch, float *d_stats, void *hip_stream) {
  if (!d_psd || !d_stats || bins < 1 || bins > 32769 || pitch < bins) return GLFER_E_ARG;
  const int m = bins - (int)(bins * 0.95);
  DeviceGuard guard(data_device(d_psd));
  HIP_TRY(guard.error());
  HIP_TRY(glfer_launch_floor(d_psd, nframes, bins, pitch, m, d_stats, (hipStream_t)hip_stream));
  return GLFER_OK;
}

int glfer_hip_floor_device(const float *d_psd, size_t nframes, int bins, float *d_stats, void *hip_stream) {
  return glfer_hip_floor_device_pitched(d_psd, nframes, bins, bins, d_stats, hip_stream);
}

int glfer_hip_avg_device(int avg_mode, const float *d_psd, size_t nframes, int bins, int n_out, int depth,
                         int minbin, int maxbin, int max0, double *d_avg, double *d_ret, void *hip_stream) {
  if (!d_psd || !d_avg || !d_ret) return GLFER_E_ARG;
  if (avg_mode < GLFER_AVG_SUMAVG || avg_mode > GLFER_AVG_SUMEXTREME) return GLFER_E_ARG;
  if (depth < 1 || minbin < 0 || maxbin <= minbin || maxbin > bins || maxbin > n_out || n_out < 1)
    return GLFER_E_ARG;
  DeviceGuard guard(data_device(d_psd));
  HIP_TRY(guard.error());
  HIP_TRY(glfer_launch_avg(avg_mode, d_psd, nframes, bins, n_out, depth, minbin, maxbin, max0 ? 1 : 0, d_avg,
                           d_ret, (hipStream_t)hip_stream));
  return GLFER_OK;
}

static bool avg_in_launch(const glfer_hip_plan *p, const SpectroParams &sp, int avg_mode, int depth, int n_out, size_t first,
                          size_t nframes, size_t *b0) {
  static const bool fused_off = [] { const char *e = getenv("GLFER_AVG_FUSED"); return e && *e == '0'; }();
  const bool with_means = p->cfg.sub_mean != 0;
  const bool fused = !fused_off && avg_mode == GLFER_AVG_PLAIN && depth <= 4 && p->cfg.mode == GLFER_MODE_FFT && !p->nonlin &&
                     !p->cfg.history_mode && p->n >= 512 && p->n <= 4096 && n_out <= 2 * p->n && body_route(sp, p->n) == ROUTE_REAL_INPUT &&
                     (!with_means || (reference_means(p) && route_takes_mean(ROUTE_REAL_INPUT, sp, p->n) && !getenv("GLFER_MEAN_PREPASS")));
  const size_t first_inside = (size_t)((p->keep + p->hop - 1) / p->hop), end = first + nframes;
  *b0 = std::max(first, first_inside) + (size_t)(depth - 1);
  return fused && *b0 + 256 <= end;
}

int glfer_hip_spectrogram_avg_device(glfer_hip_plan *p, const void *d_stream, size_t nsamples, size_t first, size_t nframes,
                                     int avg_mode, int depth, int minbin, int maxbin, int max0, int n_out, float *d_psd,
                                     double *d_avg, double *d_ret, void *hip_stream) {
  if (!p || !d_stream || (!d_avg && nframes)) return GLFER_E_ARG;
  if (p->cfg.mode == GLFER_MODE_HPARMA || p->pitch != p->bins) return GLFER_E_ARG;
  if (avg_mode < GLFER_AVG_SUMAVG || avg_mode > GLFER_AVG_SUMEXTREME) return GLFER_E_ARG;
  if (depth < 1 || minbin < 0 || maxbin <= minbin || maxbin > p->bins || n_out < p->bins) return GLFER_E_ARG;
  if (nframes == 0) return GLFER_OK;
  if ((first + nframes) > nsamples / (size_t)p->hop || nframes > 0x7fffffffu) return GLFER_E_ARG;
  hipStream_t st = (hipStream_t)hip_stream;
  DeviceGuard guard(p->cfg.device);
  HIP_TRY(guard.error());
  const size_t bins = (size_t)p->bins;
  int rc = GLFER_OK;
  auto two_launches = [&](size_t from, size_t to) {
    if (rc != GLFER_OK || from >= to) return;
    const size_t nf = to - from;
    float *rows = d_psd ? d_psd + (from - first) * bins : nullptr;
    double *ret = d_ret ? d_ret + (from - first) * 4 : nullptr;
    hipError_t e = hipSuccess;
    if (!d_psd) e = glfer::scratch_malloc((void **)&rows, nf * bins * sizeof(float), st);
    if (e == hipSuccess && !d_ret) e = glfer::scratch_malloc((void **)&ret, nf * 4 * sizeof(double), st);
    if (e != hipSuccess) rc = hip_fail(e, "scratch (rows to average)");
    if (rc == GLFER_OK) rc = glfer_run_device(p, d_stream, nsamples, from, nf, rows, nullptr, st);
    if (rc == GLFER_OK) {
      e = glfer_launch_avg(avg_mode, rows, nf, (int)bins, n_out, depth, minbin, maxbin, max0 ? 1 : 0, d_avg + (from - first) * (size_t)n_out, ret, st);
      if (e != hipSuccess) rc = hip_fail(e, "update_avg launch");
    }
    if (!d_psd && rows) glfer::scratch_free(rows, st);
// ... 206 lines not shown
```

### glfer_amd/csrc/plan.h

```cpp
#pragma once
#include "../../include/glfer_hip.h"

#include <hip/hip_runtime.h>
#include <stdint.h>

#include <string>
#include <vector>

namespace glfer {

int hip_fail(hipError_t e, const char *what);
std::string error_text();
void set_error_text(const std::string &text);

class DeviceGuard {
 public:
  explicit DeviceGuard(int device) {
    if (hipGetDevice(&prev_) != hipSuccess) prev_ = -1;
    err_ = (device == prev_) ? hipSuccess : hipSetDevice(device);
    changed_ = err_ == hipSuccess && device != prev_;
  }
  ~DeviceGuard() {
    if (changed_ && prev_ >= 0) (void)hipSetDevice(prev_);
  }
  hipError_t error() const { return err_; }
  DeviceGuard(const DeviceGuard &) = delete;
  DeviceGuard &operator=(const DeviceGuard &) = delete;

 private:
  int prev_ = -1;
  bool changed_ = false;
  hipError_t err_ = hipSuccess;
};

int device_of(const void *d_ptr);

hipError_t scratch_malloc(void **p, size_t bytes, hipStream_t st);
void scratch_free(void *p, hipStream_t st);
size_t scratch_trim(int dev, size_t keep_bytes);
size_t scratch_held(int dev);
void scratch_set_cap(size_t bytes);
bool scratch_keeping();
size_t scratch_cap();

hipError_t allow_dynamic_lds(const void *kernel, size_t bytes);

struct IngestRing {
  unsigned char *h_in[2] = {nullptr, nullptr}, *d_in[2] = {nullptr, nullptr}, *h_out[2] = {nullptr, nullptr};
  unsigned char *d_rgb[2] = {nullptr, nullptr};
  short *h_lev[2] = {nullptr, nullptr}, *d_lev[2] = {nullptr, nullptr};
  float *d_psd[2] = {nullptr, nullptr}, *d_stats[2] = {nullptr, nullptr};
  hipStream_t st[2] = {nullptr, nullptr};
  hipStream_t up = nullptr;
  hipEvent_t ev_up[2] = {nullptr, nullptr};
  hipEvent_t ev_t[2][4] = {{nullptr, nullptr, nullptr, nullptr}, {nullptr, nullptr, nullptr, nullptr}};
  size_t cap[2][8] = {{0, 0, 0, 0, 0, 0, 0, 0}, {0, 0, 0, 0, 0, 0, 0, 0}};
  bool busy = false;
};
void ingest_ring_free(IngestRing *r);
IngestRing *ingest_ring_take(int dev);
void ingest_ring_drop_spare(int dev);
void workers_drop_kept();
size_t workers_kept_bytes(int dev);
size_t ingest_ring_spare_bytes(int dev);

}

#define HIP_TRY(call)                                          \
  do {                                                         \
    hipError_t e_ = (call);                                    \
    if (e_ != hipSuccess) return glfer::hip_fail(e_, #call);   \
  } while (0)

struct glfer_hip_plan {
  glfer_hip_config cfg;
  int n, hop, keep, bins, ntapers, npairs, lanes;
  int pitch = 0;
  int lmp_av = 0;
  std::vector<float> window;
  std::vector<double> tapers;
  std::vector<double> sig;
  float *d_taps = nullptr;
  float *d_window = nullptr;
  float2 *d_tw = nullptr;
  float *d_htaps = nullptr;
  int htapers = 0;
  float2 *d_htw = nullptr;
  float2 *d_hrot = nullptr;
  float *d_wtaps = nullptr;
  int wtapers = 0;
  float2 *d_wtw = nullptr;
  float2 *d_wcomb = nullptr;
  float2 *d_bigtw = nullptr;
  float *d_xtaps = nullptr;
  float *d_ltaps = nullptr;
  uint16_t *d_lagmap = nullptr;
  int *d_rot_sched = nullptr;
  int rot_steps = 0, rot_width = 8;
  float2 *d_unit = nullptr;
  float *d_ftaps_mu_first = nullptr;
  float *d_ftaps = nullptr;
  float *d_ftaps2 = nullptr;
  float *d_ftaps2_nomu = nullptr;
  double *d_U0 = nullptr;
  std::vector<double> U0;
  std::vector<float> hn;
  float sum_U0_sqr = 0.0f;
  float hn_scale = 1.0f;
  float spec_unscale = 1.0f;
  bool nonlin = false;
  glfer::IngestRing *ring = nullptr;
  hipStream_t aux[2] = {nullptr, nullptr};
  std::vector<hipEvent_t> aux_events;
  bool aux_busy = false;
};

int glfer_run_device(glfer_hip_plan *p, const void *d_stream, size_t nsamples, size_t first, size_t nframes,
                     float *d_psd, float *d_spec, hipStream_t st, long tail_fresh = -1);
```

### glfer_amd/csrc/spectro16y.hip

```cpp
#include <hip/hip_runtime.h>
#include <stdint.h>
#include "odd_taper.hpp"

#ifndef GLFER16Y_DPP_SUM
#define GLFER16Y_DPP_SUM 1
#endif
#ifndef GLFER16Y_SKEW
#define GLFER16Y_SKEW 1
#endif
#ifndef GLFER16Y_TW1_REGS
#define GLFER16Y_TW1_REGS 1
#endif

namespace glfer {

hipError_t allow_dynamic_lds(const void *kernel, size_t bytes);

struct LaunchY {
  static constexpr int N = 4096, T = 256, PADN = N + N / 16;
  static constexpr int LDS_WORDS = 2 * PADN + 16 * 17 + 4;
};

template <int FMT, int ABL = 0, int HIST = 0, int KM = 0, int BAT = 0>
__global__ __launch_bounds__(256, 2) void spectro16y_kernel(SpectroParams p) {
  if constexpr (KM == 0 || BAT != 0) glfer_batch_select(p);
  static_assert(KM == 0 || (HIST == 0 && (KM == 16 || KM == 8 || KM == 4)), "in-kernel mean removal: history from the stream");
  constexpr int NH = KM > 0 ? 16 / KM : 1;
  __shared__ float mred[KM > 0 ? 4 * (NH + 1) : 1];
  using C = Plan16<12>;
  using L = LaunchY;
  constexpr int N = L::N, T = L::T, PADN = L::PADN, NPASS = C::NPASS;
  constexpr int TW1 = 15;
  constexpr int NT = C::NTW - TW1;
  constexpr unsigned esz = FMT == GLFER_FMT_F32 ? 4 : (FMT == GLFER_FMT_S16 ? 2 : 1);
  typedef float v4f32 __attribute__((ext_vector_type(4)));
  extern __shared__ v2f32 lds[];

  const unsigned t = threadIdx.x;
  v2f32 *xbA = lds, *xbB = lds + PADN;
  v2f32 *tw1 = lds + 2 * PADN;
  float *red = reinterpret_cast<float *>(lds + 2 * PADN + 16 * 17);

  {
    const v2f32 *tw = reinterpret_cast<const v2f32 *>(p.tw);
    const unsigned k = t >> 4, q = t & 15;
    tw1[k * 17 + q] = q ? tw[(q - 1) * T + k] : v2f32{1.0f, 0.0f};
  }
  float twr[NT], twi[NT];
  {
    const v2f32 *tw = reinterpret_cast<const v2f32 *>(p.tw) + t;
#pragma unroll
    for (int e = 0; e < NT; e++) {
      const v2f32 w = tw[(TW1 + e) * T];
      twr[e] = w.x;
      twi[e] = w.y;
    }
  }
  __syncthreads();
  const v2f32 *tw1row = tw1 + (t & 15) * 17;
  constexpr bool TW1R = GLFER16Y_TW1_REGS != 0 && HIST == 0 && KM != 4;
  v2f32 tw1reg[16];
  if constexpr (TW1R) {
#pragma unroll
    for (int q = 0; q < 16; q++) tw1reg[q] = tw1row[q];
  }

  const __amdgpu_buffer_rsrc_t trsrc = __builtin_amdgcn_make_buffer_rsrc(
      const_cast<float *>(p.taps), 0, p.npairs * 2 * N * 4, 0x00020000);
  const __amdgpu_buffer_rsrc_t vrsrc = __builtin_amdgcn_make_buffer_rsrc(
      const_cast<float *>(p.xtaps), 0, N * 4, 0x00020000);
  const unsigned toff = t * 16u;
  const int NP = p.npairs - 1;
  const long long stride = (long long)gridDim.x * 2;

  auto load_x = [&](float (&dst)[16], long long f) {
    load_frame16<FMT, T, HIST>(p, t, 0u, f < p.nframes ? f : (long long)p.nframes - 1, dst);
  };
  v2f32 pt[16];
  auto prefetch_taps = [&](int pair) {
    const unsigned tap_p = (unsigned)pair * (N * 8u);
    static_for<0, 8>([&](auto mc) {
      constexpr int mh = decltype(mc)::value;
      const v4f32 q = __builtin_bit_cast(v4f32, __builtin_amdgcn_raw_buffer_load_b128(trsrc, toff, tap_p + (unsigned)(T * mh) * 16u, 0));
      pt[2 * mh] = v2f32{q.x, q.y};
      pt[2 * mh + 1] = v2f32{q.z, q.w};
    });
  };
  auto prefetch_last = [&] {
    static_for<0, 4>([&](auto mc) {
      constexpr int mq = decltype(mc)::value;
      const v4f32 q = __builtin_bit_cast(v4f32, __builtin_amdgcn_raw_buffer_load_b128(vrsrc, toff, (unsigned)(T * mq) * 16u, 0));
      pt[2 * mq] = v2f32{q.x, q.y};
      pt[2 * mq + 1] = v2f32{q.z, q.w};
    });
  };

  long long fA = (long long)xcd_block_index() * 2;
  if (fA >= p.nframes) return;
  float xA[16], xB[16];
  load_x(xA, fA);
  if (fA + 1 < p.nframes) load_x(xB, fA + 1);
  else {
#pragma unroll
    for (int m = 0; m < 16; m++) xB[m] = 0.0f;
  }
  prefetch_taps(0);

  auto publish_hop_sums = [&] {
    static_for<0, NH + 1>([&](auto qc) {
      constexpr int q = decltype(qc)::value;
      float sm = 0.0f;
      static_for<0, KM>([&](auto mc) {
        constexpr int m = decltype(mc)::value;
        sm += q < NH ? xA[q * KM + m] : xB[(NH - 1) * KM + m];
      });
#pragma unroll
      for (int o = 1; o < 64; o <<= 1) sm += __shfl_xor(sm, o);
      if ((t & 63u) == 0) mred[(t >> 6) * (NH + 1) + q] = sm;
    });
  };
  auto subtract_hop_means = [&] {
    float mu[NH + 1];
#pragma unroll
    for (int q = 0; q <= NH; q++)
      mu[q] = ((mred[q] + mred[(NH + 1) + q]) + (mred[2 * (NH + 1) + q] + mred[3 * (NH + 1) + q])) / (float)p.H;
#pragma unroll
    for (int m = 0; m < 16; m++) {
      xA[m] = xA[m] - mu[m / (KM ? KM : 1)];
      xB[m] = xB[m] - mu[m / (KM ? KM : 1) + 1];
    }
  };
  auto subtract_table_means = [&](long long fa) {
    float mu[NH + 1];
    const long long F = p.frame0 + fa;
#pragma unroll
    for (int q = 0; q < NH; q++) mu[q] = p.means[F - (NH - 1) + q];
    mu[NH] = p.means[fa + 1 < p.nframes ? F + 1 : F];
#pragma unroll
    for (int m = 0; m < 16; m++) {
      xA[m] = xA[m] - mu[m / (KM ? KM : 1)];
      xB[m] = xB[m] - mu[m / (KM ? KM : 1) + 1];
    }
  };
  if constexpr (KM > 0) {
    if (p.means) {
      subtract_table_means(fA);
    } else {
      publish_hop_sums();
      __syncthreads();
      subtract_hop_means();
      __syncthreads();
    }
    if (fA + 1 >= p.nframes) {
#pragma unroll
      for (int m = 0; m < 16; m++) xB[m] = 0.0f;
    }
  }

  constexpr int RL = C::radix(NPASS - 1), BL = 16 / RL;
  auto rho_of = [](int m) constexpr { return (m % BL) + BL * brev(m / BL, RL); };

  while (true) {
    const long long nfA = fA + stride;
    const bool has_next = nfA < p.nframes;
    float psdA[8], psdB[8], nyqA, nyqB;
    int hxA, hxB;
    {
      float accA[16], accB[16];
#pragma unroll
      for (int r = 0; r < 16; r++) accA[r] = accB[r] = 0.0f;
      for (int pair = 0; pair < NP; pair++) {
        float zrA[16], ziA[16], zrB[16], ziB[16];
        GLFER_STAMP(0);
#pragma unroll
        for (int m = 0; m < 16; m++) {
          zrA[m] = xA[m] * pt[m].x;
          ziA[m] = xA[m] * pt[m].y;
          zrB[m] = xB[m] * pt[m].x;
          ziB[m] = xB[m] * pt[m].y;
        }
        auto dual = [&](const auto &tw1sel) {
          auto hook = [&] {
            if (pair + 1 < NP) prefetch_taps(pair + 1);
            else prefetch_last();
          };
          if constexpr (GLFER16Y_SKEW != 0) stockham16_passes2s<12, NT>(zrA, ziA, xbA, zrB, ziB, xbB, t, tw1sel, twr, twi, hook);
          else stockham16_passes2<12, NT>(zrA, ziA, xbA, zrB, ziB, xbB, t, tw1sel, twr, twi, hook);
        };
        if constexpr (TW1R) dual(tw1reg);
        else dual(tw1row);
        if (pair == 0) {
#pragma unroll
          for (int r = 0; r < 16; r++) {
            accA[r] = __builtin_fmaf(zrA[r], zrA[r], ziA[r] * ziA[r]);
            accB[r] = __builtin_fmaf(zrB[r], zrB[r], ziB[r] * ziB[r]);
          }
        } else {
#pragma unroll
          for (int r = 0; r < 16; r++) {
            accA[r] = __builtin_fmaf(zrA[r], zrA[r], __builtin_fmaf(ziA[r], ziA[r], accA[r]));
            accB[r] = __builtin_fmaf(zrB[r], zrB[r], __builtin_fmaf(ziB[r], ziB[r], accB[r]));
          }
        }
        GLFER_STAMP(15);
      }
      float eA = 0.0f, eB = 0.0f;
#pragma unroll
      for (int r = 0; r < 16; r++) {
        eA += accA[r];
        eB += accB[r];
      }
#if GLFER16Y_DPP_SUM
      eA = wave_total_f32(eA);
      eB = wave_total_f32(eB);
#else
#pragma unroll
      for (int w = 1; w < 64; w <<= 1) {
        eA += __shfl_xor(eA, w);
        eB += __shfl_xor(eB, w);
      }
#endif
      float *foldA = reinterpret_cast<float *>(xbA), *foldB = reinterpret_cast<float *>(xbB);
      static_for<8, 16>([&](auto mc) {
        constexpr int m = decltype(mc)::value;
        foldA[t + T * (m - 8)] = accA[rho_of(m)];
        foldB[t + T * (m - 8)] = accB[rho_of(m)];
      });
      if ((t & 63) == 0) {
        red[t >> 6] = eA;
        red[4 + (t >> 6)] = eB;
      }
      __syncthreads();
      eA = (red[0] + red[1]) + (red[2] + red[3]);
      eB = (red[4] + red[5]) + (red[6] + red[7]);
      hxA = scale_exponent(eA);
      hxB = scale_exponent(eB);
      static_for<0, 8>([&](auto mc) {
        constexpr int m = decltype(mc)::value;
        const int k = T * m + (int)t;
        float oa = foldA[N / 2 - k], ob = foldB[N / 2 - k];
        if constexpr (m == 0) {
          if (t == 0) {
            oa = accA[rho_of(0)];
            ob = accB[rho_of(0)];
          }
        }
        psdA[m] = accA[rho_of(m)] + oa;
        psdB[m] = accB[rho_of(m)] + ob;
      });
      nyqA = 2.0f * accA[rho_of(8)];
      nyqB = 2.0f * accB[rho_of(8)];
      __syncthreads();
    }

    if constexpr (ABL == 1) {
      if (has_next) {
        prefetch_taps(0);
        load_x(xA, nfA);
        load_x(xB, nfA + 1);
      }
      if (t == 0) p.psd[(size_t)fA * (size_t)p.pitch] = psdA[0] + psdB[0] + nyqA + nyqB + (float)(hxA + hxB);
      if (!has_next) break;
      fA = nfA;
      continue;
    }
    float zr[16], zi[16];
    GLFER_STAMP(0);
    {
      const float sA = scale_in(hxA), sB = scale_in(hxB);
#pragma unroll
      for (int m = 0; m < 16; m++) {
        const float v = (m & 1) ? pt[m / 2].y : pt[m / 2].x;
        zr[m] = (xA[m] * v) * sA;
        zi[m] = (xB[m] * v) * sB;
      }
    }
    auto shared_round = [&](const auto &tw1sel) {
      auto hook = [&] {
        if (has_next) {
          prefetch_taps(0);
          load_x(xA, nfA);
          load_x(xB, nfA + 1);
        }
      };
      if constexpr (GLFER16Y_SKEW >= 2) stockham16_passes1s<12, NT>(zr, zi, xbA, t, tw1sel, twr, twi, hook);
      else stockham16_passes<12, NT>(zr, zi, xbA, t, tw1sel, twr, twi, hook);
    };
    if constexpr (TW1R) shared_round(tw1reg);
    else shared_round(tw1row);
    if constexpr (KM > 0) {
      if (has_next && !p.means) publish_hop_sums();
    }
    separate_and_store<12, 1>(p, zr, zi, xbA, t, 0u, fA, hxA, hxB,
                              [&](auto mc) { if constexpr (decltype(mc)::value == 8) return nyqA; else return psdA[decltype(mc)::value]; },
                              [&](auto mc) { if constexpr (decltype(mc)::value == 8) return nyqB; else return psdB[decltype(mc)::value]; });
    GLFER_STAMP(15);
    if constexpr (KM > 0) {
      if (has_next) {
        if (p.means) subtract_table_means(nfA);
        else subtract_hop_means();
      }
    }
    if (!has_next) break;
    fA = nfA;
    if (fA + 1 >= p.nframes) {
#pragma unroll
      for (int m = 0; m < 16; m++) xB[m] = 0.0f;
    }
  }
}

}

#ifndef GLFER_NO_LAUNCHERS
using namespace glfer;

template <int FMT>
static hipError_t launch16y_fmt(const SpectroParams &p, hipStream_t st) {
  const long long work = ((long long)p.nframes + 1) / 2;
  if (work == 0) return hipSuccess;
  const long long resident = 256LL * 2;
  const long long cap = glfer_batch_cap(16 * resident, p.nbatch);
  unsigned grid = (unsigned)(work < cap ? work : cap);
  if (grid >= 64) grid &= ~7u;
  constexpr size_t shmem = (size_t)LaunchY::LDS_WORDS * 8;
  {
    hipError_t e = allow_dynamic_lds(reinterpret_cast<const void *>(p.history_mode ? spectro16y_kernel<FMT, 0, 1> : spectro16y_kernel<FMT, 0, 0>), shmem);
    if (e != hipSuccess) return e;
  }
  if (p.mean_inkernel) {
    if (p.history_mode) return hipErrorInvalidValue;
    const int km = p.H % 256 == 0 ? p.H / 256 : 0;
#define GLFER_Y_MEAN(K)                                                                                              \
  do {                                                                                                               \
    const void *k_ = p.nbatch > 1 ? reinterpret_cast<const void *>(spectro16y_kernel<FMT, 0, 0, K, 1>)                 \
                                  : reinterpret_cast<const void *>(spectro16y_kernel<FMT, 0, 0, K, 0>);                \
    hipError_t e = allow_dynamic_lds(k_, shmem);                                                                     \
    if (e != hipSuccess) return e;                                                                                   \
    if (p.nbatch > 1) hipLaunchKernelGGL((spectro16y_kernel<FMT, 0, 0, K, 1>), dim3(grid, glfer_batch_y(p)), dim3(256), shmem, st, p); \
    else hipLaunchKernelGGL((spectro16y_kernel<FMT, 0, 0, K, 0>), dim3(grid, 1), dim3(256), shmem, st, p);          \
    return hipGetLastError();                                                                                        \
  } while (0)
    if (km == 16) GLFER_Y_MEAN(16);
    if (km == 8) GLFER_Y_MEAN(8);
    if (km == 4) GLFER_Y_MEAN(4);
#undef GLFER_Y_MEAN
    return hipErrorInvalidValue;
  }
  if (p.history_mode) hipLaunchKernelGGL((spectro16y_kernel<FMT, 0, 1>), dim3(grid, glfer_batch_y(p)), dim3(256), shmem, st, p);
  else hipLaunchKernelGGL((spectro16y_kernel<FMT, 0, 0>), dim3(grid, glfer_batch_y(p)), dim3(256), shmem, st, p);
  return hipGetLastError();
}

extern "C" hipError_t glfer_launch_spectro16y_n12(const SpectroParams *p, hipStream_t st) {
  if (!p->xtaps || p->npairs < 2 || p->nonlin || p->spec) return hipErrorInvalidValue;
  if (p->frame0 * (long long)p->H < (long long)p->R) return hipErrorInvalidValue;
  switch (p->fmt) {
    case GLFER_FMT_F32: return launch16y_fmt<GLFER_FMT_F32>(*p, st);
    case GLFER_FMT_S16: return launch16y_fmt<GLFER_FMT_S16>(*p, st);
    case GLFER_FMT_U8: return launch16y_fmt<GLFER_FMT_U8>(*p, st);
  }
  return hipErrorInvalidValue;
}
#endif
```

### glfer_amd/csrc/spectro_params.h

```cpp
#ifndef GLFER_SPECTRO_PARAMS_H
#define GLFER_SPECTRO_PARAMS_H

#include <hip/hip_runtime.h>

enum { GLFER_FMT_F32 = 0, GLFER_FMT_S16 = 1, GLFER_FMT_U8 = 2 };

struct SpectroParams {
  const void *stream;
  long long frame0;
  int nframes;
  int H;
  int R;
  int npairs;
  int history_mode;
  int fmt;
  int nonlin;
  int limiter;
  float a;
  float post_scale;
  float spec_unscale;
  const float *taps;
  const float2 *tw;
  const float *htaps;
  const float2 *htw;
  int htapers;
  const float2 *hrot;
  const float *wtaps;
  int wtapers;
  const float2 *wtw;
  const float2 *wcomb;
  const float2 *bigtw;
  const float *xtaps;
  const float *ltaps;
  float *psd;
  int pitch;
  float *spec;
  float *ftest;
  const double *ft_U0;
  float ft_sum_U0_sqr;
  int ft_mu_live;
  int ft_nseq;
  float ft_mu_unscale;
  int mean_inkernel;
  const float *means;
  int nprod;
  int prod_chunk;
  float *means_out;
  unsigned *means_ready;
  long long prod_hop0;
  long long prod_nhops;
  long long prod_front_frames;
  int prod_block_frames;
  int prod_look;
  unsigned *front_done;
  double *avg;
  double *avg_ret;
  int avg_depth;
  int avg_minbin, avg_maxbin, avg_nout;
  int nbatch;
  long long batch_stride;
  long long psd_batch_stride;
  long long means_batch_stride;
  long long avg_batch_stride;
  long long avg_ret_batch_stride;
};

static inline long long glfer_batch_cap(long long cap, int nbatch) {
  return nbatch > 1 ? (cap + nbatch - 1) / nbatch : cap;
}
static inline unsigned glfer_batch_y(const SpectroParams &p) { return p.nbatch > 1 ? (unsigned)p.nbatch : 1u; }

#ifdef __HIPCC__
__device__ __forceinline__ void glfer_batch_select(SpectroParams &p) {
  const long long b = (long long)blockIdx.y;
  p.stream = reinterpret_cast<const char *>(p.stream) + b * p.batch_stride;
  p.psd = p.psd + b * p.psd_batch_stride;
  if (p.means) p.means = p.means + b * p.means_batch_stride;
}
__device__ __forceinline__ void glfer_batch_select_avg(SpectroParams &p) {
  glfer_batch_select(p);
  const long long b = (long long)blockIdx.y;
  p.avg = p.avg + b * p.avg_batch_stride;
  p.avg_ret = p.avg_ret + b * p.avg_ret_batch_stride;
}
#endif

#ifdef __cplusplus
extern "C" {
#endif
hipError_t glfer_launch_spectro16_n8(const SpectroParams *p, hipStream_t st);
hipError_t glfer_launch_spectro16_n9(const SpectroParams *p, hipStream_t st);
hipError_t glfer_launch_spectro16_n10(const SpectroParams *p, hipStream_t st);
hipError_t glfer_launch_spectro16_n11(const SpectroParams *p, hipStream_t st);
hipError_t glfer_launch_spectro16_n12(const SpectroParams *p, hipStream_t st);
hipError_t glfer_launch_spectro16_n13(const SpectroParams *p, hipStream_t st);
hipError_t glfer_launch_spectro16_n14(const SpectroParams *p, hipStream_t st);
hipError_t glfer_launch_spectro16x_n8(const SpectroParams *p, hipStream_t st);
hipError_t glfer_launch_spectro16x_n9(const SpectroParams *p, hipStream_t st);
hipError_t glfer_launch_spectro16x_n10(const SpectroParams *p, hipStream_t st);
hipError_t glfer_launch_spectro16xl_n8(const SpectroParams *p, hipStream_t st);
hipError_t glfer_launch_spectro16xl_n9(const SpectroParams *p, hipStream_t st);
hipError_t glfer_launch_spectro16xl_n10(const SpectroParams *p, hipStream_t st);
hipError_t glfer_launch_spectro16xl_n11(const SpectroParams *p, hipStream_t st);
hipError_t glfer_launch_spectro16y_n12(const SpectroParams *p, hipStream_t st);
hipError_t glfer_launch_spectro16h_n9(const SpectroParams *p, hipStream_t st);
hipError_t glfer_launch_spectro16h_n10(const SpectroParams *p, hipStream_t st);
hipError_t glfer_launch_spectro16h_n11(const SpectroParams *p, hipStream_t st);
hipError_t glfer_launch_spectro16h_n12(const SpectroParams *p, hipStream_t st);
hipError_t glfer_launch_spectro16h_n13(const SpectroParams *p, hipStream_t st);
hipError_t glfer_launch_spectro16h_n14(const SpectroParams *p, hipStream_t st);
hipError_t glfer_launch_spectro16w_n11(const SpectroParams *p, hipStream_t st);
hipError_t glfer_launch_spectro16w_n12(const SpectroParams *p, hipStream_t st);
hipError_t glfer_launch_spectro16w_n13(const SpectroParams *p, hipStream_t st);
hipError_t glfer_launch_spectro16w_n14(const SpectroParams *p, hipStream_t st);
size_t glfer_levels_scratch_floats(size_t nframes);
hipError_t glfer_launch_levels(const float *stats, size_t nframes, int scale_log, int autoscale,
                               int first_buffer, float overlap, float max_lvl0, float min_lvl0,
                               float *levels, float *chunk_state, hipStream_t st);
hipError_t glfer_launch_levels_fixed(size_t nframes, float dmax, float dmin, float max_lvl, float min_lvl,
                                     float *levels, hipStream_t st);
hipError_t glfer_launch_map(const float *psd, const double *avg, size_t nframes, int n, int psd_pitch, int scale_log,
                            double thr255, double one_m_thr, const float *levels,
                            const unsigned char *colortab, const double *log_thr, unsigned char *rgb, short *lev,
                            hipStream_t st);
hipError_t glfer_launch_submean(const void *in, float *out, int H, long long nhops, int fmt,
                                hipStream_t st, const float *means );
hipError_t glfer_launch_submean_batch(const void *in, float *out, int H, long long nhops, int fmt, hipStream_t st, const float *means,
                                      unsigned nb, long long in_bstride, long long out_bstride, long long means_bstride);
hipError_t glfer_launch_hop_means_seq_batch(const void *in, float *means, int H, long long nhops, int fmt, unsigned nb,
                                            long long in_bstride, long long means_bstride, hipStream_t st);
#ifdef __cplusplus
}
#endif
#endif
```

### glfer_amd/csrc/stockham16.hpp

```cpp
#pragma once
#include <hip/hip_runtime.h>
#include <stdint.h>
#include "fft_inreg.hpp"
#include "spectro_params.h"

#ifndef GLFER_STAMP
#define GLFER_STAMP(id)
#endif
#ifndef GLFER16_FOLD_TW
#define GLFER16_FOLD_TW 1
#endif
#ifndef GLFER16_BARRIER_AFTER_READS
#define GLFER16_BARRIER_AFTER_READS 1
#endif

namespace glfer {

typedef float v2f32 __attribute__((ext_vector_type(2)));

template <int LOGN>
struct Plan16 {
  static constexpr int N = 1 << LOGN;
  static constexpr int T = N / 16;
  static constexpr int NPASS = LOGN <= 8 ? 2 : (LOGN <= 12 ? 3 : 4);
// ... 4 lines not shown
  }
  static constexpr int ls(int i) {
    int l = 1;
    for (int j = 0; j < i; j++) l *= radix(j);
    return l;
  }
  static constexpr int tw_offset(int i) {
    int o = 0;
    for (int j = 1; j < i; j++) o += (16 / radix(j)) * (radix(j) - 1);
    return o;
  }
  static constexpr int NTW = tw_offset(NPASS);
};


template <int FMT>
__device__ __forceinline__ float cvt_sample(const void *ubase, unsigned elem_off) {
  if constexpr (FMT == GLFER_FMT_F32) {
    return *reinterpret_cast<const float *>(reinterpret_cast<const char *>(ubase) + (size_t)(elem_off * 4u));
  } else if constexpr (FMT == GLFER_FMT_S16) {
    return (float)*reinterpret_cast<const short *>(reinterpret_cast<const char *>(ubase) + (size_t)(elem_off * 2u)) / 32768.0f;
  } else {
    return ((float)*(reinterpret_cast<const unsigned char *>(ubase) + (size_t)elem_off) - 128.0f) / 128.0f;
  }
}

#ifndef GLFER_X_LOAD_AUX
#define GLFER_X_LOAD_AUX 0
#endif
template <int FMT>
__device__ __forceinline__ float buf_sample(__amdgpu_buffer_rsrc_t rsrc, unsigned voff_bytes, unsigned soff_bytes) {
  if constexpr (FMT == GLFER_FMT_F32) {
    return __uint_as_float(__builtin_amdgcn_raw_buffer_load_b32(rsrc, voff_bytes, soff_bytes, GLFER_X_LOAD_AUX));
  } else if constexpr (FMT == GLFER_FMT_S16) {
    return (float)(short)__builtin_amdgcn_raw_buffer_load_b16(rsrc, voff_bytes, soff_bytes, GLFER_X_LOAD_AUX) / 32768.0f;
  } else {
    return ((float)(unsigned char)__builtin_amdgcn_raw_buffer_load_b8(rsrc, voff_bytes, soff_bytes, GLFER_X_LOAD_AUX) - 128.0f) / 128.0f;
  }
}

__device__ __forceinline__ float limiter_value(float y) {
  const float ftmp = (float)log((double)fabsf(y));
  const float mag = (float)exp((double)ftmp * 0.1);
  return y > 0.0f ? mag : -mag;
}

__device__ __forceinline__ unsigned xcd_block_index() {
  const unsigned w = blockIdx.x, g = gridDim.x;
  return (g & 7u) ? w : (w & 7u) * (g >> 3) + (w >> 3);
}

#ifndef GLFER_ABL
#define GLFER_ABL 0
#endif
template <int T>
__device__ __forceinline__ void frame_sync() {
  if constexpr (T > 64 && !(GLFER_ABL & 1)) {
    __syncthreads();
  } else {
    __builtin_amdgcn_fence(__ATOMIC_ACQ_REL, "wavefront");
    __builtin_amdgcn_wave_barrier();
  }
}

template <int LOGN>
struct Launch16 {
  static constexpr int T = Plan16<LOGN>::T;
  static constexpr int FPB = T >= 256 ? 1 : 256 / T;
  static constexpr int BLOCK = T * FPB;
  static constexpr int PADN = Plan16<LOGN>::N + Plan16<LOGN>::N / 16;
  static constexpr int LDS_WORDS = FPB * PADN + 16 * 17;
};

__host__ __device__ constexpr int xpad_shift(int exchange) { return exchange == 0 ? 4 : 5; }
__host__ __device__ constexpr int xpad_offset(int exchange, int d) { return d + (d >> xpad_shift(exchange)); }

#ifndef GLFER16_X0_ROWS
#define GLFER16_X0_ROWS 1
#endif
template <int BYTE_OFFSET>
__device__ __forceinline__ void lds_read_b64_asm(unsigned addr, v2f32 &out) {
  asm volatile("ds_read_b64 %0, %1 offset:%2" : "=v"(out) : "v"(addr), "n"(BYTE_OFFSET) : "memory");
}
template <int STRIDE>
__device__ __forceinline__ void lds_read16_strided(const v2f32 *base, v2f32 (&v)[16]) {
  static_assert(15 * STRIDE * 8 < 65536, "ds offset field");
  const unsigned addr = (unsigned)(__SIZE_TYPE__)(const __attribute__((address_space(3))) char *)base;
  static_for<0, 16>([&](auto mc) {
    constexpr int m = decltype(mc)::value;
    lds_read_b64_asm<m * STRIDE * 8>(addr, v[m]);
  });
  asm volatile("s_waitcnt lgkmcnt(0)"
               : "+v"(v[0]), "+v"(v[1]), "+v"(v[2]), "+v"(v[3]), "+v"(v[4]), "+v"(v[5]), "+v"(v[6]), "+v"(v[7]), "+v"(v[8]),
                 "+v"(v[9]), "+v"(v[10]), "+v"(v[11]), "+v"(v[12]), "+v"(v[13]), "+v"(v[14]), "+v"(v[15])
               :
               : "memory");
}

template <int STRIDE>
__device__ __forceinline__ void lds_issue16_strided(const v2f32 *base, v2f32 (&v)[16]) {
  static_assert(15 * STRIDE * 8 < 65536, "ds offset field");
  const unsigned addr = (unsigned)(__SIZE_TYPE__)(const __attribute__((address_space(3))) char *)base;
  static_for<0, 16>([&](auto mc) {
    constexpr int m = decltype(mc)::value;
    lds_read_b64_asm<m * STRIDE * 8>(addr, v[m]);
  });
}
template <int K>
__device__ __forceinline__ void lds_wait16(v2f32 (&v)[16]) {
  asm volatile("s_waitcnt lgkmcnt(%16)"
               : "+v"(v[0]), "+v"(v[1]), "+v"(v[2]), "+v"(v[3]), "+v"(v[4]), "+v"(v[5]), "+v"(v[6]), "+v"(v[7]), "+v"(v[8]),
                 "+v"(v[9]), "+v"(v[10]), "+v"(v[11]), "+v"(v[12]), "+v"(v[13]), "+v"(v[14]), "+v"(v[15])
               : "n"(K)
               : "memory");
}

template <bool REGS>
struct Tw1Source {
  v2f32 r[REGS ? 16 : 1];
  const v2f32 *row;
  __device__ __forceinline__ void init(const v2f32 *tw1row) {
    row = tw1row;
    if constexpr (REGS) {
#pragma unroll
      for (int q = 0; q < 16; q++) r[q] = tw1row[q];
    }
  }
  __device__ __forceinline__ v2f32 operator[](int q) const {
    if constexpr (REGS) return r[q];
    else return row[q];
  }
};

template <class C, int I, int NT, class Tw1>
struct PassTwiddles {
  const Tw1 &tw1row;
  const float (&twr)[NT];
  const float (&twi)[NT];
  template <int M>
  __device__ __forceinline__ auto operator()(std::integral_constant<int, M>) const {
    constexpr int R = C::radix(I), B = 16 / R, b = M % B, q = M / B;
    if constexpr (I == 0 || q == 0) {
      return NoTwiddle{};
    } else if constexpr (I == 1) {
      return tw1row[M];
    } else {
      constexpr int e = C::tw_offset(I) - 15 + b * (R - 1) + (q - 1);
      return v2f32{twr[e], twi[e]};
    }
  }
};

template <int LOGM, int NT, class Tw1, class Hook>
__device__ __forceinline__ void stockham16_passes(float (&zr)[16], float (&zi)[16], v2f32 *xb, unsigned t,
                                                  const Tw1 &tw1row, const float (&twr)[NT],
                                                  const float (&twi)[NT], Hook &&after_first_write) {
  using C = Plan16<LOGM>;
  constexpr int T = C::T, NPASS = C::NPASS, TW1 = 15;
  static_for<0, NPASS>([&](auto ic) {
    constexpr int i = decltype(ic)::value;
    constexpr int R = C::radix(i), Ls = C::ls(i), B = 16 / R;
    constexpr bool kFold = GLFER16_FOLD_TW != 0 && i > 0;
    const PassTwiddles<C, i, NT, Tw1> twf{tw1row, twr, twi};
    if constexpr (kFold) {
    } else if constexpr (i == 1) {
      static_for<1, 16>([&](auto qc) {
        constexpr int q = decltype(qc)::value;
        const v2f32 w = tw1row[q];
        const float a = zr[q], c = zi[q];
        zr[q] = __builtin_fmaf(a, w.x, -c * w.y);
        zi[q] = __builtin_fmaf(a, w.y, c * w.x);
      });
    } else if constexpr (i > 1) {
      static_for<0, B>([&](auto bc) {
        constexpr int b = decltype(bc)::value;
        static_for<1, R>([&](auto qc) {
          constexpr int q = decltype(qc)::value;
          constexpr int e = C::tw_offset(i) - TW1 + b * (R - 1) + (q - 1);
          constexpr int m = b + B * q;
          const float a = zr[m], c = zi[m];
          zr[m] = __builtin_fmaf(a, twr[e], -c * twi[e]);
          zi[m] = __builtin_fmaf(a, twi[e], c * twr[e]);
        });
      });
    }
    constexpr bool kEmit = GLFER16_BARRIER_AFTER_READS != 0 && i < NPASS - 1 && B == 1;
    if constexpr (kEmit) {
      const int k = (int)t & (Ls - 1);
      const int a0 = ((int)t - k) * R + k;
      constexpr bool kRows = GLFER16_X0_ROWS != 0 && i == 0 && T >= 32;
      v2f32 *wbase = kRows ? xb + t : xb + a0 + (a0 >> xpad_shift(i));
      if constexpr (kFold) dit_head_tw<R, 1, 0, 16>(zr, zi, twf);
      else dit_head<R, 1, 0, 16>(zr, zi);
      dit_tail<R, 1, 0, 16>(zr, zi, [&](auto qc, auto rc) {
        constexpr int q = decltype(qc)::value, reg = decltype(rc)::value;
        if constexpr (!(GLFER_ABL & 2)) wbase[kRows ? q * (T + 2) : xpad_offset(i, q * Ls)] = v2f32{zr[reg], zi[reg]};
      });
    } else {
      static_for<0, B>([&](auto bc) {
        constexpr int b = decltype(bc)::value;
        if constexpr (kFold) dit_tw<R, B, b, 16>(zr, zi, twf);
        else dit<R, B, b, 16>(zr, zi);
      });
    }
    GLFER_STAMP(4 * i + 1);
    if constexpr (i < NPASS - 1) {
      if constexpr (GLFER16_BARRIER_AFTER_READS == 0) frame_sync<T>();
      GLFER_STAMP(4 * i + 2);
      if constexpr (!kEmit) static_for<0, B>([&](auto bc) {
        constexpr int b = decltype(bc)::value;
        const int j = (int)t + T * b;
        const int k = j & (Ls - 1);
        const int a0 = (j - k) * R + k;
        v2f32 *wbase = xb + a0 + (a0 >> xpad_shift(i));
        static_for<0, R>([&](auto qc) {
          constexpr int q = decltype(qc)::value;
          constexpr int src = b + B * brev(q, R);
          wbase[xpad_offset(i, q * Ls)] = v2f32{zr[src], zi[src]};
        });
      });
      if constexpr (i == 0) {
        after_first_write();
        __builtin_amdgcn_sched_barrier(0);
      }
      GLFER_STAMP(4 * i + 3);
      frame_sync<T>();
      GLFER_STAMP(4 * i + 4);
      if constexpr (GLFER_ABL & 4) {
      } else if constexpr (GLFER16_X0_ROWS != 0 && GLFER16_BARRIER_AFTER_READS != 0 && i == 0 && T >= 32 && B == 1) {
        v2f32 v[16];
        lds_read16_strided<T / 16>(xb + (t & 15) * (T + 2) + (t >> 4), v);
#pragma unroll
        for (int m = 0; m < 16; m++) {
          zr[m] = v[m].x;
          zi[m] = v[m].y;
        }
      } else {
        const v2f32 *rbase = xb + t + (t >> xpad_shift(i));
        constexpr int STRIDE = xpad_offset(i, T);
        if constexpr (GLFER16_X0_ROWS != 0 && T % 32 == 0 && i > 0 && 15 * STRIDE * 8 < 65536 && xpad_offset(i, 15 * T) == 15 * STRIDE) {
          v2f32 v[16];
          lds_read16_strided<STRIDE>(rbase, v);
#pragma unroll
          for (int m = 0; m < 16; m++) {
            zr[m] = v[m].x;
            zi[m] = v[m].y;
          }
        } else {
          static_for<0, 16>([&](auto mc) {
            constexpr int m = decltype(mc)::value;
            const v2f32 v = rbase[xpad_offset(i, m * T)];
            zr[m] = v.x;
            zi[m] = v.y;
          });
        }
      }
      if constexpr (GLFER16_BARRIER_AFTER_READS != 0) frame_sync<T>();
    }
  });
}

template <int LOGM, int NT, class Tw1, class Hook>
__device__ __forceinline__ void stockham16_passes2(float (&zrA)[16], float (&ziA)[16], v2f32 *xbA, float (&zrB)[16],
                                                   float (&ziB)[16], v2f32 *xbB, unsigned t, const Tw1 &tw1row,
                                                   const float (&twr)[NT], const float (&twi)[NT],
                                                   Hook &&after_first_write) {
  using C = Plan16<LOGM>;
  constexpr int T = C::T, NPASS = C::NPASS, TW1 = 15;
  static_assert(GLFER16_BARRIER_AFTER_READS != 0, "stockham16_passes2 relies on the barrier-after-reads scheme");
  static_for<0, NPASS>([&](auto ic) {
    constexpr int i = decltype(ic)::value;
    constexpr int R = C::radix(i), Ls = C::ls(i), B = 16 / R;
    constexpr bool kFold = GLFER16_FOLD_TW != 0 && i > 0;
    const PassTwiddles<C, i, NT, Tw1> twf{tw1row, twr, twi};
    auto compute = [&](float (&zr)[16], float (&zi)[16], v2f32 *xb) {
      if constexpr (kFold) {
      } else if constexpr (i == 1) {
        static_for<1, 16>([&](auto qc) {
          constexpr int q = decltype(qc)::value;
          const v2f32 w = tw1row[q];
          const float a = zr[q], c = zi[q];
          zr[q] = __builtin_fmaf(a, w.x, -c * w.y);
          zi[q] = __builtin_fmaf(a, w.y, c * w.x);
        });
      } else if constexpr (i > 1) {
        static_for<0, B>([&](auto bc) {
          constexpr int b = decltype(bc)::value;
          static_for<1, R>([&](auto qc) {
            constexpr int q = decltype(qc)::value;
            constexpr int e = C::tw_offset(i) - TW1 + b * (R - 1) + (q - 1);
            constexpr int m = b + B * q;
            const float a = zr[m], c = zi[m];
            zr[m] = __builtin_fmaf(a, twr[e], -c * twi[e]);
            zi[m] = __builtin_fmaf(a, twi[e], c * twr[e]);
          });
        });
      }
      if constexpr (i < NPASS - 1) {
        static_assert(B == 1, "an exchange follows radix-16 passes only");
        const int k = (int)t & (Ls - 1);
        const int a0 = ((int)t - k) * R + k;
        constexpr bool kRows = GLFER16_X0_ROWS != 0 && i == 0 && T >= 32;
        v2f32 *wbase = kRows ? xb + t : xb + a0 + (a0 >> xpad_shift(i));
        if constexpr (kFold) dit_head_tw<R, 1, 0, 16>(zr, zi, twf);
        else dit_head<R, 1, 0, 16>(zr, zi);
        dit_tail<R, 1, 0, 16>(zr, zi, [&](auto qc, auto rc) {
          constexpr int q = decltype(qc)::value, reg = decltype(rc)::value;
          if constexpr (!(GLFER_ABL & 2)) wbase[kRows ? q * (T + 2) : xpad_offset(i, q * Ls)] = v2f32{zr[reg], zi[reg]};
        });
      } else {
        static_for<0, B>([&](auto bc) {
          constexpr int b = decltype(bc)::value;
          if constexpr (kFold) dit_tw<R, B, b, 16>(zr, zi, twf);
          else dit<R, B, b, 16>(zr, zi);
        });
      }
    };
    compute(zrA, ziA, xbA);
    GLFER_STAMP(4 * i + 1);
    __builtin_amdgcn_sched_barrier(0);
    compute(zrB, ziB, xbB);
    if constexpr (i < NPASS - 1) {
      if constexpr (i == 0) after_first_write();
      __builtin_amdgcn_sched_barrier(0);
      GLFER_STAMP(4 * i + 2);
      frame_sync<T>();
      GLFER_STAMP(4 * i + 3);
      if constexpr (GLFER_ABL & 4) {
      } else if constexpr (GLFER16_X0_ROWS != 0 && i == 0 && T >= 32) {
        v2f32 va[16], vb[16];
        const int roff = (int)(t & 15) * (T + 2) + (int)(t >> 4);
        lds_read16_strided<T / 16>(xbA + roff, va);
        lds_read16_strided<T / 16>(xbB + roff, vb);
#pragma unroll
        for (int m = 0; m < 16; m++) {
          zrA[m] = va[m].x;
          ziA[m] = va[m].y;
          zrB[m] = vb[m].x;
          ziB[m] = vb[m].y;
        }
      } else {
        const v2f32 *ra = xbA + t + (t >> xpad_shift(i)), *rb = xbB + t + (t >> xpad_shift(i));
        constexpr int STRIDE = xpad_offset(i, T);
        if constexpr (GLFER16_X0_ROWS != 0 && T % 32 == 0 && i > 0 && 15 * STRIDE * 8 < 65536 && xpad_offset(i, 15 * T) == 15 * STRIDE) {
          v2f32 va[16], vb[16];
          lds_read16_strided<STRIDE>(ra, va);
          lds_read16_strided<STRIDE>(rb, vb);
#pragma unroll
          for (int m = 0; m < 16; m++) {
            zrA[m] = va[m].x;
            ziA[m] = va[m].y;
            zrB[m] = vb[m].x;
            ziB[m] = vb[m].y;
          }
        } else {
          static_for<0, 16>([&](auto mc) {
            constexpr int m = decltype(mc)::value;
            const v2f32 v = ra[xpad_offset(i, m * T)];
            zrA[m] = v.x;
            ziA[m] = v.y;
          });
          static_for<0, 16>([&](auto mc) {
            constexpr int m = decltype(mc)::value;
            const v2f32 v = rb[xpad_offset(i, m * T)];
            zrB[m] = v.x;
            ziB[m] = v.y;
          });
        }
      }
      frame_sync<T>();
      GLFER_STAMP(4 * i + 4);
    }
  });
}

template <int LOGM, int NT, class Tw1, class Hook>
__device__ __forceinline__ void stockham16_passes2s(float (&zrA)[16], float (&ziA)[16], v2f32 *xbA, float (&zrB)[16],
                                                    float (&ziB)[16], v2f32 *xbB, unsigned t, const Tw1 &tw1row,
                                                    const float (&twr)[NT], const float (&twi)[NT],
                                                    Hook &&after_first_write) {
  using C = Plan16<LOGM>;
  constexpr int T = C::T, NPASS = C::NPASS, TW1 = 15;
  static_assert(GLFER16_BARRIER_AFTER_READS != 0 && GLFER16_X0_ROWS != 0 && T >= 32 && T % 32 == 0 && !(GLFER_ABL & 7), "the product configuration");
  static_for<0, NPASS>([&](auto ic) {
    constexpr int i = decltype(ic)::value;
    constexpr int R = C::radix(i), Ls = C::ls(i);
    static_assert(R == 16, "radix-16 passes");
    constexpr bool kFold = GLFER16_FOLD_TW != 0 && i > 0;
    const PassTwiddles<C, i, NT, Tw1> twf{tw1row, twr, twi};
    auto twiddle = [&](float (&zr)[16], float (&zi)[16]) {
      if constexpr (kFold) {
        dit_head_tw<R, 1, 0, 16>(zr, zi, twf);
      } else if constexpr (i == 1) {
        static_for<1, 16>([&](auto qc) {
          constexpr int q = decltype(qc)::value;
          const v2f32 w = tw1row[q];
          const float a = zr[q], c = zi[q];
          zr[q] = __builtin_fmaf(a, w.x, -c * w.y);
          zi[q] = __builtin_fmaf(a, w.y, c * w.x);
        });
      } else if constexpr (i > 1) {
        static_for<1, R>([&](auto qc) {
          constexpr int q = decltype(qc)::value;
          constexpr int e = C::tw_offset(i) - TW1 + (q - 1);
          const float a = zr[q], c = zi[q];
          zr[q] = __builtin_fmaf(a, twr[e], -c * twi[e]);
          zi[q] = __builtin_fmaf(a, twi[e], c * twr[e]);
        });
      }
      if constexpr (!kFold) dit_head<R, 1, 0, 16>(zr, zi);
    };
    auto tail = [&](float (&zr)[16], float (&zi)[16], v2f32 *xb) {
      if constexpr (i < NPASS - 1) {
        const int k = (int)t & (Ls - 1);
        const int a0 = ((int)t - k) * R + k;
        constexpr bool kRows = i == 0;
        v2f32 *wbase = kRows ? xb + t : xb + a0 + (a0 >> xpad_shift(i));
        dit_tail<R, 1, 0, 16>(zr, zi, [&](auto qc, auto rc) {
          constexpr int q = decltype(qc)::value, reg = decltype(rc)::value;
          wbase[kRows ? q * (T + 2) : xpad_offset(i, q * Ls)] = v2f32{zr[reg], zi[reg]};
        });
      } else {
        dit_tail<R, 1, 0, 16>(zr, zi, [](auto, auto) {});
      }
    };
    if constexpr (i == 0) {
      dit_head<R, 1, 0, 16>(zrA, ziA);
      tail(zrA, ziA, xbA);
      __builtin_amdgcn_sched_barrier(0);
      dit_head<R, 1, 0, 16>(zrB, ziB);
      tail(zrB, ziB, xbB);
      after_first_write();
      __builtin_amdgcn_sched_barrier(0);
      frame_sync<T>();
    } else {
      v2f32 va[16], vb[16];
      if constexpr (i == 1) {
        const int roff = (int)(t & 15) * (T + 2) + (int)(t >> 4);
        lds_issue16_strided<T / 16>(xbA + roff, va);
        lds_issue16_strided<T / 16>(xbB + roff, vb);
      } else {
        constexpr int STRIDE = xpad_offset(i - 1, T);
        static_assert(15 * STRIDE * 8 < 65536 && xpad_offset(i - 1, 15 * T) == 15 * STRIDE, "one stride");
        lds_issue16_strided<STRIDE>(xbA + t + (t >> xpad_shift(i - 1)), va);
        lds_issue16_strided<STRIDE>(xbB + t + (t >> xpad_shift(i - 1)), vb);
      }
      lds_wait16<15>(va);
#pragma unroll
      for (int m = 0; m < 16; m++) {
        zrA[m] = va[m].x;
        ziA[m] = va[m].y;
      }
      twiddle(zrA, ziA);
      lds_wait16<0>(vb);
#pragma unroll
      for (int m = 0; m < 16; m++) {
        zrB[m] = vb[m].x;
        ziB[m] = vb[m].y;
      }
      frame_sync<T>();
      tail(zrA, ziA, xbA);
      __builtin_amdgcn_sched_barrier(0);
      twiddle(zrB, ziB);
      tail(zrB, ziB, xbB);
      if constexpr (i < NPASS - 1) {
        __builtin_amdgcn_sched_barrier(0);
        frame_sync<T>();
      }
    }
  });
}

template <int LOGM, int NT, class Tw1, class Hook>
__device__ __forceinline__ void stockham16_passes1s(float (&zr)[16], float (&zi)[16], v2f32 *xb, unsigned t, const Tw1 &tw1row,
                                                    const float (&twr)[NT], const float (&twi)[NT], Hook &&after_first_write) {
  using C = Plan16<LOGM>;
  constexpr int T = C::T, NPASS = C::NPASS, TW1 = 15;
  static_assert(GLFER16_BARRIER_AFTER_READS != 0 && GLFER16_X0_ROWS != 0 && T >= 32 && T % 32 == 0 && !(GLFER_ABL & 7), "the product configuration");
  static_for<0, NPASS>([&](auto ic) {
    constexpr int i = decltype(ic)::value;
    constexpr int R = C::radix(i), Ls = C::ls(i);
    static_assert(R == 16, "radix-16 passes");
    auto tail = [&] {
      if constexpr (i < NPASS - 1) {
        const int k = (int)t & (Ls - 1);
        const int a0 = ((int)t - k) * R + k;
        constexpr bool kRows = i == 0;
        v2f32 *wbase = kRows ? xb + t : xb + a0 + (a0 >> xpad_shift(i));
        dit_tail<R, 1, 0, 16>(zr, zi, [&](auto qc, auto rc) {
          constexpr int q = decltype(qc)::value, reg = decltype(rc)::value;
          wbase[kRows ? q * (T + 2) : xpad_offset(i, q * Ls)] = v2f32{zr[reg], zi[reg]};
        });
      } else {
        dit_tail<R, 1, 0, 16>(zr, zi, [](auto, auto) {});
      }
    };
    if constexpr (i == 0) {
      dit_head<R, 1, 0, 16>(zr, zi);
      tail();
      after_first_write();
      __builtin_amdgcn_sched_barrier(0);
      frame_sync<T>();
    } else {
      v2f32 v[16];
      if constexpr (i == 1) {
        lds_read16_strided<T / 16>(xb + (t & 15) * (T + 2) + (t >> 4), v);
      } else {
        constexpr int STRIDE = xpad_offset(i - 1, T);
        static_assert(15 * STRIDE * 8 < 65536 && xpad_offset(i - 1, 15 * T) == 15 * STRIDE, "one stride");
        lds_read16_strided<STRIDE>(xb + t + (t >> xpad_shift(i - 1)), v);
      }
#pragma unroll
      for (int m = 0; m < 16; m++) {
        zr[m] = v[m].x;
        zi[m] = v[m].y;
      }
      if constexpr (GLFER16_FOLD_TW != 0) {
        const PassTwiddles<C, i, NT, Tw1> twf{tw1row, twr, twi};
        dit_head_tw<R, 1, 0, 16>(zr, zi, twf);
      } else {
        if constexpr (i == 1) {
          static_for<1, 16>([&](auto qc) {
            constexpr int q = decltype(qc)::value;
            const v2f32 w = tw1row[q];
            const float a = zr[q], c = zi[q];
            zr[q] = __builtin_fmaf(a, w.x, -c * w.y);
            zi[q] = __builtin_fmaf(a, w.y, c * w.x);
          });
        } else {
          static_for<1, R>([&](auto qc) {
            constexpr int q = decltype(qc)::value;
            constexpr int e = C::tw_offset(i) - TW1 + (q - 1);
            const float a = zr[q], c = zi[q];
            zr[q] = __builtin_fmaf(a, twr[e], -c * twi[e]);
            zi[q] = __builtin_fmaf(a, twi[e], c * twr[e]);
          });
        }
        dit_head<R, 1, 0, 16>(zr, zi);
      }
      frame_sync<T>();
      tail();
      if constexpr (i < NPASS - 1) {
        __builtin_amdgcn_sched_barrier(0);
        frame_sync<T>();
      }
    }
  });
}

}
```

### include/glfer_hip.h

```cpp
#ifndef GLFER_HIP_H
#define GLFER_HIP_H

#include <stddef.h>

#ifdef __cplusplus
extern "C" {
#endif

#define GLFER_MODE_FFT 0
#define GLFER_MODE_MTM 1
#define GLFER_MODE_HPARMA 2
#define GLFER_MODE_LMP 3

#define GLFER_WIN_HANNING 0
#define GLFER_WIN_BLACKMAN 1
#define GLFER_WIN_GAUSSIAN 2
#define GLFER_WIN_WELCH 3
#define GLFER_WIN_BARTLETT 4
#define GLFER_WIN_RECTANGULAR 5
#define GLFER_WIN_HAMMING 6
#define GLFER_WIN_KAISER 7

#define GLFER_SAMPLES_F32 0
#define GLFER_SAMPLES_S16 1
#define GLFER_SAMPLES_U8 2

#define GLFER_HISTORY_ZERO_FIRST 0
#define GLFER_HISTORY_ZERO_ALWAYS 1

#define GLFER_AVG_SUMAVG 1
#define GLFER_AVG_PLAIN 2
#define GLFER_AVG_SUMEXTREME 3

#define GLFER_OK 0
#define GLFER_E_ARG (-1)
#define GLFER_E_HIP (-2)
#define GLFER_E_NOMEM (-3)
#define GLFER_E_NUMERIC (-4)

typedef struct glfer_hip_config {
  int mode;
  int n;
  float overlap;
  int window_type;
  float limiter_a;
  int enable_limiter;
  int sub_mean;
  int history_mode;
  float mtm_w;
  int mtm_k;
  int sample_format;
  int device;
  int hparma_t;
  int hparma_p_e;
  int lmp_av;
  int psd_pitch;
} glfer_hip_config;

enum { GLFER_SUBMEAN_OFF = 0, GLFER_SUBMEAN_EXACT = 1, GLFER_SUBMEAN_FAST = 2 };
#define GLFER_HIP_ABI 5
int glfer_hip_abi_version(void);

#define GLFER_FRAME_ALIGN 32
void glfer_hip_frame_range(size_t total_frames, unsigned rank, unsigned world, size_t *first, size_t *count);

typedef struct glfer_hip_plan glfer_hip_plan;

int glfer_hip_plan_create(const glfer_hip_config *cfg, glfer_hip_plan **plan_out);
void glfer_hip_plan_destroy(glfer_hip_plan *plan);

int glfer_hip_hop(const glfer_hip_plan *plan);
int glfer_hip_bins(const glfer_hip_plan *plan);
int glfer_hip_num_tapers(const glfer_hip_plan *plan);
size_t glfer_hip_num_frames(const glfer_hip_plan *plan, size_t nsamples);

int glfer_hip_get_window(const glfer_hip_plan *plan, float *window);
int glfer_hip_get_tapers(const glfer_hip_plan *plan, double *tapers, double *sig);

int glfer_hip_make_window(int window_type, int n, float *window);
int glfer_hip_make_dpss(int n, int kmax, double nw, double *tapers, double *sig);

int glfer_hip_spectrogram_device(glfer_hip_plan *plan, const void *d_stream, size_t nsamples,
                                 size_t first_frame, size_t nframes, float *d_psd,
                                 void *hip_stream);

int glfer_hip_spectrogram_batch_device(glfer_hip_plan *plan, const void *d_streams, size_t nstreams,
                                       size_t stream_pitch, size_t nsamples, size_t first_frame,
                                       size_t nframes, float *d_psd, void *hip_stream);


int glfer_hip_spectrum_device(glfer_hip_plan *plan, const void *d_stream, size_t nsamples,
                              size_t first_frame, size_t nframes, float *d_psd, float *d_spec,
                              void *hip_stream);

int glfer_hip_prepare_device(glfer_hip_plan *plan, const void *d_stream, size_t nsamples,
                             size_t first_frame, size_t nframes, float *d_frames, void *hip_stream);

int glfer_hip_mtm_ftest_device(glfer_hip_plan *plan, const void *d_stream, size_t nsamples,
                               size_t first_frame, size_t nframes, float *d_ftest, int mu_live,
                               void *hip_stream);

int glfer_hip_spectrogram_host(glfer_hip_plan *plan, const void *h_stream, size_t nsamples,
                               float *h_psd, size_t *nframes_out);

void *glfer_hip_host_alloc(size_t bytes);
void glfer_hip_host_free(void *p);

int glfer_hip_spectrogram_host_multi(const glfer_hip_config *cfg, unsigned device_mask,
                                     const void *h_stream, size_t nsamples, float *h_psd,
                                     size_t *nframes_out);
int glfer_hip_numa_node_of_bus_id(const char *bus_id, const char *sysfs_root);
int glfer_hip_numa_node_cpus(int node, const char *sysfs_root, unsigned char *mask, size_t mask_bytes);

int glfer_hip_spectrogram_host_workers(const glfer_hip_config *cfg, const int *devices, int nworkers,
                                       const void *h_stream, size_t nsamples, float *h_psd,
                                       size_t *nframes_out);

typedef struct glfer_wav_info {
  int format;
  int channels;
  int sample_rate;
  int bits_per_sample;
  size_t data_offset;
  size_t nsamples;
  size_t data_bytes;
} glfer_wav_info;
int glfer_hip_wav_probe(const char *path, glfer_wav_info *info);

int glfer_hip_spectrogram_wav(glfer_hip_plan *plan, const char *path, float *h_psd, size_t max_frames,
                              size_t *nframes_out, size_t chunk_frames);
#define GLFER_WAV_PARTIAL_TAIL 1u
int glfer_hip_spectrogram_wav_ex(glfer_hip_plan *plan, const char *path, float *h_psd, size_t max_frames,
                                 size_t *nframes_out, size_t chunk_frames, unsigned flags);

int glfer_hip_spectrogram_wav_range(glfer_hip_plan *plan, const char *path, size_t first_frame, size_t max_frames,
                                    float *h_psd, size_t *nframes_out, size_t chunk_frames, unsigned flags);

int glfer_hip_spectrogram_wav_multi(const glfer_hip_config *cfg, unsigned device_mask, const char *path, float *h_psd,
                                    size_t max_frames, size_t *nframes_out, unsigned flags);
int glfer_hip_spectrogram_wav_workers(const glfer_hip_config *cfg, const int *devices, int nworkers, const char *path,
                                      float *h_psd, size_t max_frames, size_t *nframes_out, unsigned flags);

typedef struct glfer_hip_phases {
  double setup_s, read_s, h2d_s, kernel_s, d2h_s, wall_s;
  unsigned chunks;
} glfer_hip_phases;
typedef struct glfer_hip_workers glfer_hip_workers;
int glfer_hip_workers_create(const glfer_hip_config *cfg, const int *devices, int nworkers, size_t hint_frames,
                             glfer_hip_workers **out);
void glfer_hip_workers_destroy(glfer_hip_workers *w);
int glfer_hip_workers_spectrogram_wav(glfer_hip_workers *w, const char *path, float *h_psd, size_t max_frames,
                                      size_t *nframes_out, unsigned flags, glfer_hip_phases *phases);
int glfer_hip_workers_spectrogram_host(glfer_hip_workers *w, const void *h_stream, size_t nsamples, float *h_psd,
                                       size_t *nframes_out, glfer_hip_phases *phases);

int glfer_hip_submean_device(const void *d_in, float *d_out, int hop, size_t nhops, int sample_format,
                             void *hip_stream);
int glfer_hip_submean_exact_device(const void *d_in, float *d_out, int hop, size_t nhops, int sample_format,
                                   void *hip_stream);

int glfer_hip_floor_device(const float *d_psd, size_t nframes, int bins, float *d_stats,
                           void *hip_stream);
int glfer_hip_floor_device_pitched(const float *d_psd, size_t nframes, int bins, int pitch, float *d_stats,
                                   void *hip_stream);

int glfer_hip_avg_device(int avg_mode, const float *d_psd, size_t nframes, int bins, int n_out,
                         int depth, int minbin, int maxbin, int max0, double *d_avg,
                         double *d_ret, void *hip_stream);
int glfer_hip_spectrogram_avg_device(glfer_hip_plan *plan, const void *d_stream, size_t nsamples, size_t first_frame,
                                     size_t nframes, int avg_mode, int depth, int minbin, int maxbin, int max0, int n_out,
                                     float *d_psd, double *d_avg, double *d_ret, void *hip_stream);

int glfer_hip_avg_batch_device(int avg_mode, const float *d_psd, size_t nstreams, size_t nframes, int bins, int n_out,
                               int depth, int minbin, int maxbin, int max0, double *d_avg, double *d_ret, void *hip_stream);

int glfer_hip_spectrogram_avg_batch_device(glfer_hip_plan *plan, const void *d_streams, size_t nstreams, size_t stream_pitch,
                                           size_t nsamples, size_t first_frame, size_t nframes, int avg_mode, int depth,
                                           int minbin, int maxbin, int max0, int n_out, float *d_psd, double *d_avg,
                                           double *d_ret, void *hip_stream);

int glfer_hip_avg_cum_device(const float *d_psd, size_t nframes, int bins, int n_out, int depth,
                             int minbin, int maxbin, double *d_cum, void *hip_stream);

enum { GLFER_SCALE_LIN = 0, GLFER_SCALE_LIN_MAX0, GLFER_SCALE_LOG, GLFER_SCALE_LOG_MAX0 };
enum { GLFER_PAL_HSV = 0, GLFER_PAL_THRESH, GLFER_PAL_COOL, GLFER_PAL_HOT, GLFER_PAL_BW,
       GLFER_PAL_BONE, GLFER_PAL_COPPER, GLFER_PAL_OTD };

typedef struct {
  int scale_type;
  int autoscale;
  float overlap;
  float max_level_db;
  float min_level_db;
  float thr_level;
  int palette;
  int first_buffer;
  float display_max_lvl;
  float display_min_lvl;
  int psd_pitch;
} glfer_hip_display;

int glfer_hip_palette(int palette, unsigned char colortab[768]);

int glfer_hip_display_device(glfer_hip_display *disp, const float *d_psd, const double *d_avg,
                             const float *d_stats, size_t nframes, int bins, unsigned char *d_rgb,
                             short *d_lev, float *d_levels, void *hip_stream);

int glfer_hip_waterfall_device(glfer_hip_display *disp, int avg_mode, int depth, int minbin, int maxbin,
                               int max0, const float *d_psd, size_t nframes, int bins,
                               unsigned char *d_rgb, short *d_lev, float *d_stats, void *hip_stream);

int glfer_hip_waterfall_batch_device(glfer_hip_display *disps, size_t nstreams, int avg_mode, int depth, int minbin, int maxbin,
                                     int max0, const float *d_psd, size_t nframes, int bins, unsigned char *d_rgb, short *d_lev,
                                     float *d_stats, void *hip_stream);

int glfer_hip_levels_host(glfer_hip_display *disp, const float *h_stats, size_t nframes, float *h_levels, int device);
int glfer_hip_waterfall_map_device(const glfer_hip_display *disp, int avg_mode, int depth, int minbin, int maxbin,
                                   int max0, const float *d_batch, size_t first, size_t nframes, int bins,
                                   const float *d_levels, unsigned char *d_rgb, short *d_lev, void *hip_stream);

int glfer_hip_waterfall_host(glfer_hip_plan *plan, glfer_hip_display *disp, const void *h_stream,
                             size_t nsamples, unsigned char *h_rgb, short *h_lev, size_t *nframes_out);

int glfer_hip_waterfall_host_workers(const glfer_hip_config *cfg, const int *devices, int nworkers,
                                     glfer_hip_display *disp, int avg_mode, int depth, int minbin, int maxbin, int max0,
                                     const void *h_stream, size_t nsamples, unsigned char *h_rgb, short *h_lev,
                                     size_t *nframes_out);
int glfer_hip_waterfall_wav_workers(const glfer_hip_config *cfg, const int *devices, int nworkers,
                                    glfer_hip_display *disp, int avg_mode, int depth, int minbin, int maxbin, int max0,
                                    const char *path, size_t max_frames, unsigned char *h_rgb, short *h_lev,
                                    size_t *nframes_out, unsigned flags);
int glfer_hip_waterfall_wav_multi(const glfer_hip_config *cfg, unsigned device_mask, glfer_hip_display *disp,
                                  int avg_mode, int depth, int minbin, int maxbin, int max0, const char *path,
                                  size_t max_frames, unsigned char *h_rgb, short *h_lev, size_t *nframes_out,
// ... 15 lines not shown
```

Baseline: 84.63 million.

## Use symmetric half taper tables held in registers for the N=4096 multitaper kernel

For N=4096 with five DPSS tapers, builds a per-lane half table that exploits the even/odd symmetry of the tapers. Each lane loads its taper values into registers once at kernel start and rebuilds the mirrored half with DPP lane swaps, instead of re-fetching taper pairs from global memory for every frame. Threads are remapped to residue columns so that mirrored points land in neighbouring lanes, which is threaded through the Stockham passes as a separate column index. The cost is higher register pressure and extra DPP and negate operations. An environment variable forces the old full-table path.

New measurement: 89.53 million (median of 6 runs). 1.06x the previous value.

```diff
diff --git a/glfer_amd/api.py b/glfer_amd/api.py
--- a/glfer_amd/api.py
+++ b/glfer_amd/api.py
@@ -18,7 +18,7 @@
 EXPORTS = [
     "glfer_hip_plan_create", "glfer_hip_plan_destroy", "glfer_hip_hop", "glfer_hip_bins",
     "glfer_hip_num_tapers", "glfer_hip_num_frames", "glfer_hip_get_window", "glfer_hip_get_tapers",
-    "glfer_hip_make_window", "glfer_hip_make_dpss", "glfer_hip_spectrogram_device",
+    "glfer_hip_make_window", "glfer_hip_make_dpss", "glfer_hip_y_half_tables", "glfer_hip_spectrogram_device",
     "glfer_hip_spectrum_device", "glfer_hip_spectrogram_host", "glfer_hip_wav_probe",
     "glfer_hip_spectrogram_wav", "glfer_hip_submean_device",
     "glfer_hip_floor_device",
@@ -109,6 +109,8 @@
     L.glfer_hip_get_tapers.argtypes = [vp, vp, vp]
     L.glfer_hip_make_window.argtypes = [C.c_int, C.c_int, vp]
     L.glfer_hip_make_dpss.argtypes = [C.c_int, C.c_int, C.c_double, vp, vp]
+    if hasattr(L, "glfer_hip_y_half_tables"):
+        L.glfer_hip_y_half_tables.argtypes = [C.c_int, C.c_int, C.c_double, vp, vp, vp]
     L.glfer_hip_spectrogram_device.argtypes = [vp, vp, sz, sz, sz, vp, vp]
     L.glfer_hip_spectrogram_batch_device.argtypes = [vp, vp, sz, sz, sz, sz, sz, vp, vp]
     L.glfer_hip_spectrum_device.argtypes = [vp, vp, sz, sz, sz, vp, vp, vp]
diff --git a/glfer_amd/csrc/glfer_hip.cpp b/glfer_amd/csrc/glfer_hip.cpp
--- a/glfer_amd/csrc/glfer_hip.cpp
+++ b/glfer_amd/csrc/glfer_hip.cpp
@@ -325,6 +325,44 @@
   return (size_t)pair * n * 2 + ((size_t)(m / 2) * T + t) * 4 + (size_t)(m & 1) * 2 + which;
 }
 
+static bool build_y_half_table(int n, const float *taps, const float *xtaps, float *half) {
+  if (n != 4096) return false;
+  const int T = n / 16;
+  auto last = [&](int i) { return xtaps[((size_t)((i / T) / 4) * T + (size_t)(i % T)) * 4 + (size_t)((i / T) & 3)]; };
+  for (int i = 0; i < n / 2; i++) {
+    for (int j = 0; j < 4; j++) {
+      const float a = taps[tap_slot(n, j / 2, i, j & 1)], b = taps[tap_slot(n, j / 2, n - 1 - i, j & 1)];
+      if (!((j & 1) ? b == -a : b == a)) return false;
+    }
+    if (!(last(n - 1 - i) == last(i))) return false;
+  }
+  for (int t = 0; t < T; t++) {
+    const int r = (int)glfer_yhalf_residue((unsigned)t);
+    float *row = half + (size_t)t * GLFER_YHALF_FLOATS;
+    for (int m = 0; m < 8; m++) {
+      for (int j = 0; j < 4; j++) row[16 * (j / 2) + 2 * m + (j & 1)] = taps[tap_slot(n, j / 2, r + T * m, j & 1)];
+      row[32 + m] = last(r + T * m);
+    }
+  }
+  return true;
+}
+
+static void mtm_pair_tables(int n, int ntapers, const double *tapers, const double *sig, float *taps) {
+  for (int j = 0; j < ntapers; j++) {
+    const double scale = std::sqrt(1.0 / (2.0 * n * (1.0 + sig[j])));
+    for (int i = 0; i < n; i++)
+      taps[tap_slot(n, j / 2, i, j & 1)] = (float)(tapers[(size_t)j * n + i] * scale);
+  }
+}
+static void mtm_last_table(int n, int ntapers, const double *tapers, const double *sig, float *xtaps) {
+  const int T = n / 16, j = ntapers - 1;
+  const double scale = std::sqrt(1.0 / (4.0 * n * (1.0 + sig[j])));
+  for (int i = 0; i < n; i++) {
+    const int t = i % T, m = i / T;
+    xtaps[((size_t)(m / 4) * T + t) * 4 + (size_t)(m & 3)] = (float)(tapers[(size_t)j * n + i] * scale);
+  }
+}
+
 extern "C" {
 
 const char *glfer_hip_version(void) { return "glfer_hip 0.9 (gfx950; 16 points/lane Stockham radix-16 with LDS exchange, inter-pass twiddles folded into the butterflies: packed pairs, real-input and wavefront-private forms, shared odd taper, register reuse across overlapped frames, mean removal in the reference's summation order (cfg.sub_mean = 1) or inside the kernels; N = 8..1048576; periodogram, multitaper + F-test, HP-ARMA with column-disjoint Jacobi rotations side by side and frames from a queue, LMP; rows at a caller's pitch; wavefront floor, fused average, display map with the average taken inside it; chunk ring for ingest with uploads and downloads at once, WAV files and waterfalls over several GPUs, read-ahead behind the per-hop shim, kept scratch blocks with a cap, workers bound to their GPU's NUMA node)"; }
@@ -868,11 +906,7 @@
       }
     }
     taps.assign((size_t)2 * p->npairs * n, 0.0f);
-    for (int j = 0; j < p->ntapers && !huge; j++) {
-      const double scale = std::sqrt(1.0 / (2.0 * n * (1.0 + p->sig[j])));
-      for (int i = 0; i < n; i++)
-        taps[tap_slot(n, j / 2, i, j & 1)] = (float)(p->tapers[(size_t)j * n + i] * scale);
-    }
+    if (!huge) mtm_pair_tables(n, p->ntapers, p->tapers.data(), p->sig.data(), taps.data());
     p->spec_unscale = 1.0f;
   }
   int logn = 0;
@@ -950,13 +984,14 @@
 
   std::vector<float> xtaps;
   if (cfg->mode == GLFER_MODE_MTM && (p->ntapers & 1) && p->ntapers >= 3 && !small && !huge) {
-    const int T = n / 16, j = p->ntapers - 1;
-    const double scale = std::sqrt(1.0 / (4.0 * n * (1.0 + p->sig[j])));
     xtaps.resize((size_t)n);
-    for (int i = 0; i < n; i++) {
-      const int t = i % T, m = i / T;
-      xtaps[((size_t)(m / 4) * T + t) * 4 + (size_t)(m & 3)] = (float)(p->tapers[(size_t)j * n + i] * scale);
-    }
+    mtm_last_table(n, p->ntapers, p->tapers.data(), p->sig.data(), xtaps.data());
+  }
+
+  std::vector<float> ytaps;
+  if (!xtaps.empty() && n == 4096 && p->ntapers == 5) {
+    ytaps.resize((size_t)(n / 16) * GLFER_YHALF_FLOATS);
+    if (!build_y_half_table(n, taps.data(), xtaps.data(), ytaps.data())) ytaps.clear();
   }
 
   std::vector<float> ltaps;
@@ -1089,6 +1124,10 @@
     e = hipMalloc((void **)&p->d_xtaps, xtaps.size() * sizeof(float));
     if (e == hipSuccess) e = hipMemcpy(p->d_xtaps, xtaps.data(), xtaps.size() * sizeof(float), hipMemcpyHostToDevice);
   }
+  if (e == hipSuccess && !ytaps.empty()) {
+    e = hipMalloc((void **)&p->d_ytaps, ytaps.size() * sizeof(float));
+    if (e == hipSuccess) e = hipMemcpy(p->d_ytaps, ytaps.data(), ytaps.size() * sizeof(float), hipMemcpyHostToDevice);
+  }
   if (e == hipSuccess && !ltaps.empty()) {
     e = hipMalloc((void **)&p->d_ltaps, ltaps.size() * sizeof(float));
     if (e == hipSuccess) e = hipMemcpy(p->d_ltaps, ltaps.data(), ltaps.size() * sizeof(float), hipMemcpyHostToDevice);
@@ -1131,6 +1170,7 @@
   if (p->d_wcomb) (void)hipFree(p->d_wcomb);
   if (p->d_bigtw) (void)hipFree(p->d_bigtw);
   if (p->d_ltaps) (void)hipFree(p->d_ltaps);
+  if (p->d_ytaps) (void)hipFree(p->d_ytaps);
   if (p->d_lagmap) (void)hipFree(p->d_lagmap);
   if (p->d_rot_sched) (void)hipFree(p->d_rot_sched);
   if (p->d_unit) (void)hipFree(p->d_unit);
@@ -1165,6 +1205,19 @@
   if (!window || n < 2 || window_type < 0 || window_type > 7) return GLFER_E_ARG;
   glfer::make_window(window_type, n, window);
   return GLFER_OK;
+}
+
+int glfer_hip_y_half_tables(int n, int kmax, double nw, float *half, float *pairs, float *last) {
+  if (!half || n != 4096 || kmax != 4 || !(nw > 0.0)) return GLFER_E_ARG;
+  const int nt = kmax + 1;
+  std::vector<double> tapers((size_t)nt * n), sig(nt);
+  if (!glfer::make_dpss(n, kmax, nw, tapers.data(), sig.data())) return GLFER_E_NUMERIC;
+  std::vector<float> taps((size_t)2 * ((nt + 1) / 2) * n, 0.0f), xtaps((size_t)n);
+  mtm_pair_tables(n, nt, tapers.data(), sig.data(), taps.data());
+  mtm_last_table(n, nt, tapers.data(), sig.data(), xtaps.data());
+  if (pairs) memcpy(pairs, taps.data(), (size_t)4 * n * sizeof(float));
+  if (last) memcpy(last, xtaps.data(), (size_t)n * sizeof(float));
+  return build_y_half_table(n, taps.data(), xtaps.data(), half) ? 1 : 0;
 }
 
 int glfer_hip_make_dpss(int n, int kmax, double nw, double *tapers, double *sig) {
@@ -1225,8 +1278,20 @@
   return e && *e ? (int)*e : 0;
 }
 
+static bool y_full_tables_forced() {
+  const char *e = getenv("GLFER_Y_TAPERS");
+  return e && !strcmp(e, "full");
+}
+
 static hipError_t launch_shared_odd(const SpectroParams &sp, int n, hipStream_t st) {
-  if (n == 4096) return glfer_launch_spectro16y_n12(&sp, st);
+  if (n == 4096) {
+    if (sp.ytaps && y_full_tables_forced()) {
+      SpectroParams q = sp;
+      q.ytaps = nullptr;
+      return glfer_launch_spectro16y_n12(&q, st);
+    }
+    return glfer_launch_spectro16y_n12(&sp, st);
+  }
   if (sp.ltaps) {
     switch (n) {
       case 256: return glfer_launch_spectro16xl_n8(&sp, st);
@@ -1349,6 +1414,7 @@
   sp.hrot = p->d_hrot;
   sp.xtaps = p->d_xtaps;
   sp.ltaps = p->d_ltaps;
+  sp.ytaps = p->d_ytaps;
   sp.wtaps = p->d_wtaps;
   sp.wtapers = p->wtapers;
   sp.wtw = p->d_wtw;
@@ -1910,7 +1976,7 @@
   sp.nonlin = 0;
   sp.post_scale = sp.spec_unscale = 1.0f;
   sp.htaps = nullptr;
-  sp.xtaps = sp.ltaps = nullptr;
+  sp.xtaps = sp.ltaps = sp.ytaps = nullptr;
   float *scratch = nullptr;
   int rc = GLFER_OK;
   if (p->cfg.sub_mean) {
diff --git a/glfer_amd/csrc/plan.h b/glfer_amd/csrc/plan.h
--- a/glfer_amd/csrc/plan.h
+++ b/glfer_amd/csrc/plan.h
@@ -94,6 +94,7 @@
   float2 *d_bigtw = nullptr;
   float *d_xtaps = nullptr;
   float *d_ltaps = nullptr;
+  float *d_ytaps = nullptr;
   uint16_t *d_lagmap = nullptr;
   int *d_rot_sched = nullptr;
   int rot_steps = 0, rot_width = 8;
diff --git a/glfer_amd/csrc/spectro16y.hip b/glfer_amd/csrc/spectro16y.hip
--- a/glfer_amd/csrc/spectro16y.hip
+++ b/glfer_amd/csrc/spectro16y.hip
@@ -7,6 +7,9 @@
 #endif
 #ifndef GLFER16Y_SKEW
 #define GLFER16Y_SKEW 1
+#endif
+#ifndef GLFER16Y_HALF
+#define GLFER16Y_HALF 1
 #endif
 #ifndef GLFER16Y_TW1_REGS
 #define GLFER16Y_TW1_REGS 1
@@ -21,10 +24,11 @@
   static constexpr int LDS_WORDS = 2 * PADN + 16 * 17 + 4;
 };
 
-template <int FMT, int ABL = 0, int HIST = 0, int KM = 0, int BAT = 0>
+template <int FMT, int ABL = 0, int HIST = 0, int KM = 0, int BAT = 0, int HALF = 0>
 __global__ __launch_bounds__(256, 2) void spectro16y_kernel(SpectroParams p) {
   if constexpr (KM == 0 || BAT != 0) glfer_batch_select(p);
   static_assert(KM == 0 || (HIST == 0 && (KM == 16 || KM == 8 || KM == 4)), "in-kernel mean removal: history from the stream");
+  static_assert(HALF == 0 || (KM == 0 && GLFER16_X0_ROWS != 0 && GLFER16_BARRIER_AFTER_READS != 0), "half tables: the plain forms, row layout of exchange 0");
   constexpr int NH = KM > 0 ? 16 / KM : 1;
   __shared__ float mred[KM > 0 ? 4 * (NH + 1) : 1];
   using C = Plan16<12>;
@@ -37,6 +41,7 @@
   extern __shared__ v2f32 lds[];
 
   const unsigned t = threadIdx.x;
+  const unsigned rc = HALF ? glfer_yhalf_residue(t) : t;
   v2f32 *xbA = lds, *xbB = lds + PADN;
   v2f32 *tw1 = lds + 2 * PADN;
   float *red = reinterpret_cast<float *>(lds + 2 * PADN + 16 * 17);
@@ -74,7 +79,7 @@
   const long long stride = (long long)gridDim.x * 2;
 
   auto load_x = [&](float (&dst)[16], long long f) {
-    load_frame16<FMT, T, HIST>(p, t, 0u, f < p.nframes ? f : (long long)p.nframes - 1, dst);
+    load_frame16<FMT, T, HIST>(p, rc, 0u, f < p.nframes ? f : (long long)p.nframes - 1, dst);
   };
   v2f32 pt[16];
   auto prefetch_taps = [&](int pair) {
@@ -95,6 +100,39 @@
     });
   };
 
+  v2f32 hp[16];
+  float hl[8];
+  const __amdgpu_buffer_rsrc_t yrsrc = __builtin_amdgcn_make_buffer_rsrc(
+      const_cast<float *>(p.ytaps), 0, HALF ? T * GLFER_YHALF_FLOATS * 4 : 0, 0x00020000);
+  const unsigned yoff = t * (unsigned)(GLFER_YHALF_FLOATS * 4);
+  auto load_half_last = [&] {
+    static_for<0, 2>([&](auto cc) {
+      constexpr int c = decltype(cc)::value;
+      const v4f32 q = __builtin_bit_cast(v4f32, __builtin_amdgcn_raw_buffer_load_b128(yrsrc, yoff, 128u + c * 16u, 0));
+      hl[4 * c] = q.x;
+      hl[4 * c + 1] = q.y;
+      hl[4 * c + 2] = q.z;
+      hl[4 * c + 3] = q.w;
+    });
+  };
+  if constexpr (HALF != 0) {
+    static_for<0, 8>([&](auto cc) {
+      constexpr int c = decltype(cc)::value;
+      const v4f32 q = __builtin_bit_cast(v4f32, __builtin_amdgcn_raw_buffer_load_b128(yrsrc, yoff, c * 16u, 0));
+      hp[2 * c] = v2f32{q.x, q.y};
+      hp[2 * c + 1] = v2f32{q.z, q.w};
+    });
+    if constexpr (HALF == 1) load_half_last();
+  }
+  auto mirror = [](float v) {
+    return __int_as_float(__builtin_amdgcn_update_dpp(0, __float_as_int(v), 0x140, 0xf, 0xf, true));
+  };
+  auto half_pair = [&](auto pc, auto mc) {
+    constexpr int P = decltype(pc)::value, m = decltype(mc)::value;
+    if constexpr (m < 8) return hp[P * 8 + m];
+    else return v2f32{mirror(hp[P * 8 + 15 - m].x), -mirror(hp[P * 8 + 15 - m].y)};
+  };
+
   long long fA = (long long)xcd_block_index() * 2;
   if (fA >= p.nframes) return;
   float xA[16], xB[16];
@@ -104,7 +142,7 @@
 #pragma unroll
     for (int m = 0; m < 16; m++) xB[m] = 0.0f;
   }
-  prefetch_taps(0);
+  if constexpr (HALF == 0) prefetch_taps(0);
 
   auto publish_hop_sums = [&] {
     static_for<0, NH + 1>([&](auto qc) {
@@ -169,6 +207,40 @@
       float accA[16], accB[16];
 #pragma unroll
       for (int r = 0; r < 16; r++) accA[r] = accB[r] = 0.0f;
+      if constexpr (HALF != 0) {
+        static_for<0, 2>([&](auto pc) {
+          constexpr int P = decltype(pc)::value;
+          float zrA[16], ziA[16], zrB[16], ziB[16];
+          GLFER_STAMP(0);
+          static_for<0, 16>([&](auto mc) {
+            constexpr int m = decltype(mc)::value;
+            const v2f32 w = half_pair(pc, mc);
+            zrA[m] = xA[m] * w.x;
+            ziA[m] = xA[m] * w.y;
+            zrB[m] = xB[m] * w.x;
+            ziB[m] = xB[m] * w.y;
+          });
+          auto dual = [&](const auto &tw1sel) {
+            auto hook = [] {};
+            if constexpr (GLFER16Y_SKEW != 0) stockham16_passes2s<12, NT>(zrA, ziA, xbA, zrB, ziB, xbB, t, rc, tw1sel, twr, twi, hook);
+            else stockham16_passes2<12, NT>(zrA, ziA, xbA, zrB, ziB, xbB, t, rc, tw1sel, twr, twi, hook);
+          };
+          if constexpr (TW1R) dual(tw1reg);
+          else dual(tw1row);
+#pragma unroll
+          for (int r = 0; r < 16; r++) {
+            if constexpr (P == 0) {
+              accA[r] = __builtin_fmaf(zrA[r], zrA[r], ziA[r] * ziA[r]);
+              accB[r] = __builtin_fmaf(zrB[r], zrB[r], ziB[r] * ziB[r]);
+            } else {
+              accA[r] = __builtin_fmaf(zrA[r], zrA[r], __builtin_fmaf(ziA[r], ziA[r], accA[r]));
+              accB[r] = __builtin_fmaf(zrB[r], zrB[r], __builtin_fmaf(ziB[r], ziB[r], accB[r]));
+            }
+          }
+          GLFER_STAMP(15);
+        });
+        if constexpr (HALF == 2) load_half_last();
+      } else
       for (int pair = 0; pair < NP; pair++) {
         float zrA[16], ziA[16], zrB[16], ziB[16];
         GLFER_STAMP(0);
@@ -255,7 +327,7 @@
 
     if constexpr (ABL == 1) {
       if (has_next) {
-        prefetch_taps(0);
+        if constexpr (HALF == 0) prefetch_taps(0);
         load_x(xA, nfA);
         load_x(xB, nfA + 1);
       }
@@ -268,23 +340,34 @@
     GLFER_STAMP(0);
     {
       const float sA = scale_in(hxA), sB = scale_in(hxB);
-#pragma unroll
-      for (int m = 0; m < 16; m++) {
-        const float v = (m & 1) ? pt[m / 2].y : pt[m / 2].x;
-        zr[m] = (xA[m] * v) * sA;
-        zi[m] = (xB[m] * v) * sB;
+      if constexpr (HALF != 0) {
+        static_for<0, 16>([&](auto mc) {
+          constexpr int m = decltype(mc)::value;
+          float v;
+          if constexpr (m < 8) v = hl[m];
+          else v = mirror(hl[15 - m]);
+          zr[m] = (xA[m] * v) * sA;
+          zi[m] = (xB[m] * v) * sB;
+        });
+      } else {
+#pragma unroll
+        for (int m = 0; m < 16; m++) {
+          const float v = (m & 1) ? pt[m / 2].y : pt[m / 2].x;
+          zr[m] = (xA[m] * v) * sA;
+          zi[m] = (xB[m] * v) * sB;
+        }
       }
     }
     auto shared_round = [&](const auto &tw1sel) {
       auto hook = [&] {
         if (has_next) {
-          prefetch_taps(0);
+          if constexpr (HALF == 0) prefetch_taps(0);
           load_x(xA, nfA);
           load_x(xB, nfA + 1);
         }
       };
-      if constexpr (GLFER16Y_SKEW >= 2) stockham16_passes1s<12, NT>(zr, zi, xbA, t, tw1sel, twr, twi, hook);
-      else stockham16_passes<12, NT>(zr, zi, xbA, t, tw1sel, twr, twi, hook);
+      if constexpr (GLFER16Y_SKEW >= 2) stockham16_passes1s<12, NT>(zr, zi, xbA, t, rc, tw1sel, twr, twi, hook);
+      else stockham16_passes<12, NT>(zr, zi, xbA, t, rc, tw1sel, twr, twi, hook);
     };
     if constexpr (TW1R) shared_round(tw1reg);
     else shared_round(tw1row);
@@ -347,6 +430,18 @@
 #undef GLFER_Y_MEAN
     return hipErrorInvalidValue;
   }
+  if (GLFER16Y_HALF != 0 && p.ytaps && p.npairs == 3) {
+#define GLFER_Y_HALF(HIST)                                                                                           \
+  do {                                                                                                               \
+    hipError_t e = allow_dynamic_lds(reinterpret_cast<const void *>(spectro16y_kernel<FMT, 0, HIST, 0, 0, GLFER16Y_HALF>), shmem); \
+    if (e != hipSuccess) return e;                                                                                   \
+    hipLaunchKernelGGL((spectro16y_kernel<FMT, 0, HIST, 0, 0, GLFER16Y_HALF>), dim3(grid, glfer_batch_y(p)), dim3(256), shmem, st, p); \
+    return hipGetLastError();                                                                                        \
+  } while (0)
+    if (p.history_mode) GLFER_Y_HALF(1);
+    else GLFER_Y_HALF(0);
+#undef GLFER_Y_HALF
+  }
   if (p.history_mode) hipLaunchKernelGGL((spectro16y_kernel<FMT, 0, 1>), dim3(grid, glfer_batch_y(p)), dim3(256), shmem, st, p);
   else hipLaunchKernelGGL((spectro16y_kernel<FMT, 0, 0>), dim3(grid, glfer_batch_y(p)), dim3(256), shmem, st, p);
   return hipGetLastError();
diff --git a/glfer_amd/csrc/spectro_params.h b/glfer_amd/csrc/spectro_params.h
--- a/glfer_amd/csrc/spectro_params.h
+++ b/glfer_amd/csrc/spectro_params.h
@@ -32,6 +32,7 @@
   const float2 *bigtw;
   const float *xtaps;
   const float *ltaps;
+  const float *ytaps;
   float *psd;
   int pitch;
   float *spec;
@@ -64,6 +65,12 @@
   long long avg_batch_stride;
   long long avg_ret_batch_stride;
 };
+
+enum { GLFER_YHALF_FLOATS = 40 };
+static inline __host__ __device__ unsigned glfer_yhalf_residue(unsigned t) {
+  const unsigned j = t >> 4, p = t & 15u;
+  return p < 8u ? 8u * j + p : 240u - 8u * j + p;
+}
 
 static inline long long glfer_batch_cap(long long cap, int nbatch) {
   return nbatch > 1 ? (cap + nbatch - 1) / nbatch : cap;
diff --git a/glfer_amd/csrc/stockham16.hpp b/glfer_amd/csrc/stockham16.hpp
--- a/glfer_amd/csrc/stockham16.hpp
+++ b/glfer_amd/csrc/stockham16.hpp
@@ -180,7 +180,7 @@
 };
 
 template <int LOGM, int NT, class Tw1, class Hook>
-__device__ __forceinline__ void stockham16_passes(float (&zr)[16], float (&zi)[16], v2f32 *xb, unsigned t,
+__device__ __forceinline__ void stockham16_passes(float (&zr)[16], float (&zi)[16], v2f32 *xb, unsigned t, unsigned col0,
                                                   const Tw1 &tw1row, const float (&twr)[NT],
                                                   const float (&twi)[NT], Hook &&after_first_write) {
   using C = Plan16<LOGM>;
@@ -217,7 +217,7 @@
       const int k = (int)t & (Ls - 1);
       const int a0 = ((int)t - k) * R + k;
       constexpr bool kRows = GLFER16_X0_ROWS != 0 && i == 0 && T >= 32;
-      v2f32 *wbase = kRows ? xb + t : xb + a0 + (a0 >> xpad_shift(i));
+      v2f32 *wbase = kRows ? xb + col0 : xb + a0 + (a0 >> xpad_shift(i));
       if constexpr (kFold) dit_head_tw<R, 1, 0, 16>(zr, zi, twf);
       else dit_head<R, 1, 0, 16>(zr, zi);
       dit_tail<R, 1, 0, 16>(zr, zi, [&](auto qc, auto rc) {
@@ -290,7 +290,7 @@
 
 template <int LOGM, int NT, class Tw1, class Hook>
 __device__ __forceinline__ void stockham16_passes2(float (&zrA)[16], float (&ziA)[16], v2f32 *xbA, float (&zrB)[16],
-                                                   float (&ziB)[16], v2f32 *xbB, unsigned t, const Tw1 &tw1row,
+                                                   float (&ziB)[16], v2f32 *xbB, unsigned t, unsigned col0, const Tw1 &tw1row,
                                                    const float (&twr)[NT], const float (&twi)[NT],
                                                    Hook &&after_first_write) {
   using C = Plan16<LOGM>;
@@ -329,7 +329,7 @@
         const int k = (int)t & (Ls - 1);
         const int a0 = ((int)t - k) * R + k;
         constexpr bool kRows = GLFER16_X0_ROWS != 0 && i == 0 && T >= 32;
-        v2f32 *wbase = kRows ? xb + t : xb + a0 + (a0 >> xpad_shift(i));
+        v2f32 *wbase = kRows ? xb + col0 : xb + a0 + (a0 >> xpad_shift(i));
         if constexpr (kFold) dit_head_tw<R, 1, 0, 16>(zr, zi, twf);
         else dit_head<R, 1, 0, 16>(zr, zi);
         dit_tail<R, 1, 0, 16>(zr, zi, [&](auto qc, auto rc) {
@@ -404,7 +404,7 @@
 
 template <int LOGM, int NT, class Tw1, class Hook>
 __device__ __forceinline__ void stockham16_passes2s(float (&zrA)[16], float (&ziA)[16], v2f32 *xbA, float (&zrB)[16],
-                                                    float (&ziB)[16], v2f32 *xbB, unsigned t, const Tw1 &tw1row,
+                                                    float (&ziB)[16], v2f32 *xbB, unsigned t, unsigned col0, const Tw1 &tw1row,
                                                     const float (&twr)[NT], const float (&twi)[NT],
                                                     Hook &&after_first_write) {
   using C = Plan16<LOGM>;
@@ -443,7 +443,7 @@
         const int k = (int)t & (Ls - 1);
         const int a0 = ((int)t - k) * R + k;
         constexpr bool kRows = i == 0;
-        v2f32 *wbase = kRows ? xb + t : xb + a0 + (a0 >> xpad_shift(i));
+        v2f32 *wbase = kRows ? xb + col0 : xb + a0 + (a0 >> xpad_shift(i));
         dit_tail<R, 1, 0, 16>(zr, zi, [&](auto qc, auto rc) {
           constexpr int q = decltype(qc)::value, reg = decltype(rc)::value;
           wbase[kRows ? q * (T + 2) : xpad_offset(i, q * Ls)] = v2f32{zr[reg], zi[reg]};
@@ -500,7 +500,7 @@
 }
 
 template <int LOGM, int NT, class Tw1, class Hook>
-__device__ __forceinline__ void stockham16_passes1s(float (&zr)[16], float (&zi)[16], v2f32 *xb, unsigned t, const Tw1 &tw1row,
+__device__ __forceinline__ void stockham16_passes1s(float (&zr)[16], float (&zi)[16], v2f32 *xb, unsigned t, unsigned col0, const Tw1 &tw1row,
                                                     const float (&twr)[NT], const float (&twi)[NT], Hook &&after_first_write) {
   using C = Plan16<LOGM>;
   constexpr int T = C::T, NPASS = C::NPASS, TW1 = 15;
@@ -514,7 +514,7 @@
         const int k = (int)t & (Ls - 1);
         const int a0 = ((int)t - k) * R + k;
         constexpr bool kRows = i == 0;
-        v2f32 *wbase = kRows ? xb + t : xb + a0 + (a0 >> xpad_shift(i));
+        v2f32 *wbase = kRows ? xb + col0 : xb + a0 + (a0 >> xpad_shift(i));
         dit_tail<R, 1, 0, 16>(zr, zi, [&](auto qc, auto rc) {
           constexpr int q = decltype(qc)::value, reg = decltype(rc)::value;
           wbase[kRows ? q * (T + 2) : xpad_offset(i, q * Ls)] = v2f32{zr[reg], zi[reg]};
@@ -576,4 +576,27 @@
   });
 }
 
-}
+template <int LOGM, int NT, class Tw1, class Hook>
+__device__ __forceinline__ void stockham16_passes(float (&zr)[16], float (&zi)[16], v2f32 *xb, unsigned t, const Tw1 &tw1row,
+                                                  const float (&twr)[NT], const float (&twi)[NT], Hook &&after_first_write) {
+  stockham16_passes<LOGM, NT>(zr, zi, xb, t, t, tw1row, twr, twi, after_first_write);
+}
+template <int LOGM, int NT, class Tw1, class Hook>
+__device__ __forceinline__ void stockham16_passes1s(float (&zr)[16], float (&zi)[16], v2f32 *xb, unsigned t, const Tw1 &tw1row,
+                                                    const float (&twr)[NT], const float (&twi)[NT], Hook &&after_first_write) {
+  stockham16_passes1s<LOGM, NT>(zr, zi, xb, t, t, tw1row, twr, twi, after_first_write);
+}
+template <int LOGM, int NT, class Tw1, class Hook>
+__device__ __forceinline__ void stockham16_passes2(float (&zrA)[16], float (&ziA)[16], v2f32 *xbA, float (&zrB)[16],
+                                                   float (&ziB)[16], v2f32 *xbB, unsigned t, const Tw1 &tw1row,
+                                                   const float (&twr)[NT], const float (&twi)[NT], Hook &&after_first_write) {
+  stockham16_passes2<LOGM, NT>(zrA, ziA, xbA, zrB, ziB, xbB, t, t, tw1row, twr, twi, after_first_write);
+}
+template <int LOGM, int NT, class Tw1, class Hook>
+__device__ __forceinline__ void stockham16_passes2s(float (&zrA)[16], float (&ziA)[16], v2f32 *xbA, float (&zrB)[16],
+                                                    float (&ziB)[16], v2f32 *xbB, unsigned t, const Tw1 &tw1row,
+                                                    const float (&twr)[NT], const float (&twi)[NT], Hook &&after_first_write) {
+  stockham16_passes2s<LOGM, NT>(zrA, ziA, xbA, zrB, ziB, xbB, t, t, tw1row, twr, twi, after_first_write);
+}
+
+}
diff --git a/include/glfer_hip.h b/include/glfer_hip.h
--- a/include/glfer_hip.h
+++ b/include/glfer_hip.h
@@ -80,6 +80,8 @@
 int glfer_hip_make_window(int window_type, int n, float *window);
 int glfer_hip_make_dpss(int n, int kmax, double nw, double *tapers, double *sig);
 
+int glfer_hip_y_half_tables(int n, int kmax, double nw, float *half, float *pairs, float *last);
+
 int glfer_hip_spectrogram_device(glfer_hip_plan *plan, const void *d_stream, size_t nsamples,
                                  size_t first_frame, size_t nframes, float *d_psd,
                                  void *hip_stream);
```
